# baurst/liso

Hardware: AMD Instinct MI355X
Metric: LISO train-step frames/sec (120k-pt clouds) (higher is better)
Workload: dtype bf16 (detector, BASELINE configs[2]) + f32 via bf16x3 MFMA (SLIM); north_star's 1e-3 on logits / flow is met by `parity_leg` (f32 via bf16x3 MFMA everywhere) and `fp32_exact_leg`, not by the bf16 detector

## Files before the change

include/liso_box_mining.h:

```cpp
#ifndef LISO_BOX_MINING_H
#define LISO_BOX_MINING_H

#include <stddef.h>
#include <stdint.h>

#ifdef __cplusplus
extern "C" {
#endif

size_t liso_scan_workspace_bytes(int batch, long n);
int liso_scan_inclusive_i32(const int32_t* in, int batch, long n, int32_t* out, void* workspace, size_t workspace_bytes,
                            void* stream);

int liso_mine_boxes_from_regions(const double* props, int batch, int k, const float* row_coords, int gx, const float* col_coords,
                                 int gy, float ppm_x, float ppm_y, float* center, double* dims, double* rot, float* dims_f32,
                                 float* rot_f32, void* stream);

typedef struct {
    int batch, k;
    int min_points;
    double aspect_ratio_max;
    double max_box_len_m;
    double min_box_area_m2;
    double min_box_volume_m3;
    int park_invalid;
} liso_mine_filter_cfg;

int liso_mine_filter_compact(const liso_mine_filter_cfg* cfg, const int64_t* num_labels, const float* center, const double* dims2,
                             const double* rot_in, const int64_t* num_pts, const float* fit_z, const float* fit_h, float* pos,
                             double* dims, double* rot, double* probs, double* velo, uint8_t* valid, int32_t* class_id,
                             int32_t* difficulty, int32_t* counts, float* kabsch_pos, float* kabsch_dims, float* kabsch_rot,
                             void* stream);

int liso_mine_box_motion(const double* trafos, int batch, int s, const float* pos, double* rot, double* velo, void* stream);

size_t liso_mine_nms_workspace_bytes(int batch, int k);
int liso_mine_nms_prepare(int batch, int k, int pre_nms_max, float* pos, double* dims, double* rot, double* probs, double* velo,
                          uint8_t* valid, int32_t* class_id, int32_t* difficulty, float* dense, uint8_t* enters, void* workspace,
                          size_t workspace_bytes, void* stream);

int liso_mine_nms_finish(int b, int k, int max_boxes, const int64_t* keep, const int32_t* num, const uint8_t* enters, float* pos,
                         double* dims, double* rot, double* probs, double* velo, uint8_t* valid, int32_t* class_id,
                         int32_t* difficulty, float* t_pos, float* t_dims, float* t_rot, uint8_t* t_valid, void* stream);

#ifdef __cplusplus
}
#endif
#endif
```

include/liso_flow_cluster.h:

```cpp
#ifndef LISO_FLOW_CLUSTER_H
#define LISO_FLOW_CLUSTER_H

#include <stddef.h>
#include <stdint.h>

#ifdef __cplusplus
extern "C" {
#endif

size_t liso_bev_dynamic_flow_workspace_bytes(int batch, int h, int w);

int liso_bev_dynamic_flow_f32(const float* points, int point_stride, const uint8_t* valid, const int32_t* pillar_coors,
                              const float* flow, int flow_stride, const double* odom_minus_eye, int batch, int n, int h,
                              int w, float* dynamicness, float* nonrigid_flow, void* workspace, size_t workspace_bytes,
                              void* stream);

int liso_odom_inverse_minus_eye_f64(const double* odom, int batch, double* out, void* stream);

size_t liso_fit_box_z_workspace_bytes(int n_points, int n_boxes);

int liso_fit_box_z_f32(const float* points, int point_stride, int n, const float* box_pos, int pos_dims,
                       const float* box_dims, int dims_dims, const float* box_rot, int k, float box_height,
                       int64_t* num_pts, float* fitted_z, float* fitted_height, void* workspace, size_t workspace_bytes,
                       void* stream);

typedef struct {
    int batch, gx, gy;
    int window;
    int min_samples;
    float eps;
    float flow_weight;
} liso_dbscan_cfg;

int liso_dbscan_components(const liso_dbscan_cfg* cfg, const uint8_t* dynamic_mask, const float* row_coords,
                           const float* col_coords, const float* flow, uint8_t* core, int32_t* parent, int32_t* is_root,
                           void* stream);

int liso_dbscan_labels(const liso_dbscan_cfg* cfg, const uint8_t* dynamic_mask, const float* row_coords, const float* col_coords,
                       const float* flow, const uint8_t* core, const int32_t* parent, const int32_t* root_rank,
                       int32_t* labels, void* stream);

int liso_region_props(const int32_t* labels, int batch, int gx, int gy, int max_labels, uint64_t* moments, double* props,
                      void* stream);

size_t liso_region_props_workspace_bytes(int batch, int gx, int gy, int max_labels);
int liso_region_props_ws(const int32_t* labels, int batch, int gx, int gy, int max_labels, uint64_t* moments, double* props,
                         void* workspace, size_t workspace_bytes, void* stream);

#ifdef __cplusplus
}
#endif
#endif
```

liso_amd/_lib.py:

```python
import ctypes
import os

import torch

_HERE = os.path.dirname(os.path.abspath(__file__))
LIB_PATH = os.path.join(_HERE, "libliso_hip.so")

_lib = None


class LisoHipError(RuntimeError):
    pass


_ERRORS = {-1: "LISO_EINVAL (bad pointer/size)", -2: "LISO_EWORKSPACE (workspace too small)",
           -3: "LISO_ELAUNCH (HIP launch failed)", -4: "LISO_GROUND_ELENGTH (int(67 / delta_R) > 255)"}


def _preload_torch_hip_runtime():
    tl = os.path.join(os.path.dirname(torch.__file__), "lib", "libamdhip64.so")
    if os.path.exists(tl):
        ctypes.CDLL(tl, mode=ctypes.RTLD_GLOBAL)


def lib():
    global _lib
    if _lib is None:
        if not os.path.exists(LIB_PATH):
            raise LisoHipError(
                f"{LIB_PATH} not found: build it with `python -c 'import __graft_entry__ as g; g.build()'` "
                "or `make -C liso_amd/csrc`.  liso_amd has no CPU fallback for device ops.")
        _preload_torch_hip_runtime()
        _lib = ctypes.CDLL(LIB_PATH)
        _declare(_lib)
    return _lib


def check(code, what):
    if code != 0:
        raise LisoHipError(f"{what} failed: {_ERRORS.get(code, code)}")


def stream_ptr(device=None):
    return ctypes.c_void_p(torch.cuda.current_stream(device).cuda_stream)


def ptr(t):
    return ctypes.c_void_p(t.data_ptr())


def multi_copy(pairs):
    import torch

    fast = []
    for d, s_ in pairs:
        if (d.is_cuda and s_.is_cuda and d.device == s_.device and d.dtype == s_.dtype and d.shape == s_.shape and d.is_contiguous()
                and s_.is_contiguous() and (not fast or fast[0][0].device == d.device)):
            if d.numel() and d.data_ptr() != s_.data_ptr():
                fast.append((d, s_))
        else:
            d.copy_(s_, non_blocking=True)
    if len(fast) == 1:
        fast[0][0].copy_(fast[0][1], non_blocking=True)
    elif fast:
        n = len(fast)
        dst = (ctypes.c_void_p * n)(*[d.data_ptr() for d, _ in fast])
        src = (ctypes.c_void_p * n)(*[s_.data_ptr() for _, s_ in fast])
        nb = (ctypes.c_size_t * n)(*[d.numel() * d.element_size() for d, _ in fast])
        with torch.cuda.device(fast[0][0].device):
            check(lib().liso_multi_copy(n, dst, src, nb, stream_ptr()), "multi_copy")


def copy_blocks(jobs):
    import torch

    n = len(jobs)
    if n == 0:
        return
    dst = (ctypes.c_void_p * n)()
    src = (ctypes.c_void_p * n)()
    rows = (ctypes.c_uint * n)()
    rb = (ctypes.c_uint * n)()
    ds = (ctypes.c_size_t * n)()
    ss = (ctypes.c_size_t * n)()

    def rows_view(t):
        assert t.dtype == torch.float32 and t.is_cuda
        if t.dim() == 1:
            assert t.stride(0) == 1 or t.numel() <= 1
            return 1, t.numel(), t.numel()
        inner = 1
        for k in range(t.dim() - 1, 0, -1):
            assert t.shape[k] == 1 or t.stride(k) == inner, (tuple(t.shape), t.stride())
            inner *= t.shape[k]
        return t.shape[0], inner, (t.stride(0) if t.shape[0] > 1 else inner)

    for i, (d, s_) in enumerate(jobs):
        assert tuple(d.shape) == tuple(s_.shape), (tuple(d.shape), tuple(s_.shape))
        r, c, dstr = rows_view(d)
        r2, c2, sstr = rows_view(s_)
        assert (r, c) == (r2, c2)
        dst[i], src[i], rows[i], rb[i], ds[i], ss[i] = d.data_ptr(), s_.data_ptr(), r, 4 * c, 4 * dstr, 4 * sstr
    with torch.cuda.device(jobs[0][0].device):
        check(lib().liso_multi_copy_rows(n, dst, src, rows, rb, ds, ss, stream_ptr()), "multi_copy_rows")


def require_cuda(*tensors):
    for t in tensors:
        if not t.is_cuda:
            raise LisoHipError("device op called with a CPU tensor; liso_amd has no CPU fallback")


_vp, _i, _f, _sz, _lg = ctypes.c_void_p, ctypes.c_int, ctypes.c_float, ctypes.c_size_t, ctypes.c_long

SIGNATURES = {
    "liso_iou3d_overlap_bev_f32": (_i, [_vp, _i, _vp, _i, _vp, _vp]),
    "liso_iou3d_iou_bev_f32": (_i, [_vp, _i, _vp, _i, _vp, _vp]),
    "liso_iou3d_nms_workspace_bytes": (_sz, [_i]),
    "liso_iou3d_nms_f32": (_i, [_vp, _i, _f, _vp, _vp, _vp, _sz, _vp]),
    "liso_iou3d_nms_normal_f32": (_i, [_vp, _i, _f, _vp, _vp, _vp, _sz, _vp]),
    "liso_iou3d_iou_bev_cpu_f32": (_i, [_vp, _i, _vp, _i, _vp]),
    "liso_pillars_voxelize_workspace_bytes": (_sz, [_vp, _i, _i]),
    "liso_pillars_voxelize_f32": (_i, [_vp, _vp, _i, _vp, _vp, _vp, _vp, _vp, _vp, _vp, _sz, _vp]),
    "liso_pfn_partials_bytes": (_sz, []),
    "liso_pfn_decorate_workspace_bytes": (_sz, [_i, _i]),
    "liso_pfn_decorate_f32": (_i, [_vp, _vp, _i, _vp, _vp, _vp, _vp, _vp, _vp, _vp, _vp, _sz, _vp]),
    "liso_pfn_bn_prepare_f32": (_i, [_vp, _vp, _vp, _i, _vp, _vp, _vp, _vp, _vp, _vp, _f, _f, _i, _vp, _vp, _vp, _vp]),
    "liso_pfn_forward_scatter": (_i, [_vp, _vp, _vp, _vp, _i, _vp, _vp, _vp, _vp, _i, _vp, _vp]),
    "liso_pfn_backward": (_i, [_vp, _vp, _vp, _vp, _i, _vp, _vp, _vp, _vp, _vp, _i, _vp, _i, _vp, _vp, _vp, _vp, _vp]),
    "liso_kabsch_workspace_bytes": (_sz, [_vp]),
    "liso_kabsch_trafos_f32": (_i, [_vp, _vp, _vp, _vp, _vp, _vp, _vp, _vp, _vp, _vp, _vp, _sz, _vp]),
    "liso_kabsch_trafos_counted_f32": (_i, [_vp, _vp, _vp, _vp, _vp, _vp, _vp, _vp, _vp, _vp, _vp, _vp, _sz, _vp]),
    "liso_symm_ortho_fwd_f64": (_i, [_vp, _i, _vp, _vp, _vp, _vp, _vp]),
    "liso_symm_ortho_bwd_f64": (_i, [_vp, _vp, _vp, _vp, _i, _vp, _vp]),
    "liso_weighted_moments_workspace_bytes": (_sz, [_i]),
    "liso_weighted_moments_fwd_f32": (_i, [_vp, _vp, _vp, _i, ctypes.c_long, _vp, _vp, _sz, _vp]),
    "liso_weighted_moments_bwd_f32": (_i, [_vp, _vp, _vp, _i, ctypes.c_long, _vp, _vp, _vp, _vp, _vp]),
    "liso_bev_dynamic_flow_workspace_bytes": (_sz, [_i, _i, _i]),
    "liso_bev_dynamic_flow_f32": (_i, [_vp, _i, _vp, _vp, _vp, _i, _vp, _i, _i, _i, _i, _vp, _vp, _vp, _sz, _vp]),
    "liso_odom_inverse_minus_eye_f64": (_i, [_vp, _i, _vp, _vp]),
    "liso_fit_box_z_workspace_bytes": (_sz, [_i, _i]),
    "liso_fit_box_z_f32": (_i, [_vp, _i, _i, _vp, _i, _vp, _i, _vp, _i, _f, _vp, _vp, _vp, _vp, _sz, _vp]),
    "liso_dbscan_components": (_i, [_vp, _vp, _vp, _vp, _vp, _vp, _vp, _vp, _vp]),
    "liso_dbscan_labels": (_i, [_vp, _vp, _vp, _vp, _vp, _vp, _vp, _vp, _vp, _vp]),
    "liso_region_props": (_i, [_vp, _i, _i, _i, _i, _vp, _vp, _vp]),
    "liso_region_props_workspace_bytes": (_sz, [_i, _i, _i, _i]),
    "liso_region_props_ws": (_i, [_vp, _i, _i, _i, _i, _vp, _vp, _vp, _sz, _vp]),
    "liso_corr_lookup_fwd_f32": (_i, [_vp, _vp, _vp, _vp, _vp, _vp]),
    "liso_corr_lookup_fwd_tiled_f32": (_i, [_vp, _vp, _vp, _vp, _vp, _vp]),
    "liso_corr_lookup_bwd_dvol_f32": (_i, [_vp, _vp, _vp, _vp, _vp]),
    "liso_corr_pyramid_fwd_f32": (_i, [_vp, _vp, _vp, _vp]),
    "liso_corr_pyramid_bwd_f32": (_i, [_vp, _vp, _vp, _vp]),
    "liso_corr_bwd_features_workspace_bytes": (_sz, [_vp]),
    "liso_corr_bwd_features_f32": (_i, [_vp, _i, _vp, _vp, _vp, _vp, _vp, _vp, _sz, _vp]),
    "liso_rows_combine_f32": (_i, [_lg, _i, _vp, _lg, _vp, _lg, _vp, _lg, _vp, _lg, _vp, _lg, _i, _vp]),
    "liso_gru_out_rows_train_f32": (_i, [_lg, _i, _vp, _lg, _vp, _vp, _lg, _vp, _lg, _vp]),
    "liso_gru_out_rows_bwd_f32": (_i, [_lg, _i, _vp, _lg, _vp, _vp, _lg, _vp, _lg, _vp, _lg, _vp, _vp, _vp]),
    "liso_gru_in_rows_bwd_f32": (_i, [_lg, _i, _vp, _lg, _vp, _lg, _vp, _vp, _vp, _lg, _vp, _lg, _vp, _vp]),
    "liso_raft_state_step_train_f32": (_i, [_i, _i, _vp, _vp, _vp, _vp, _vp, _vp, _vp, _vp, _vp]),
    "liso_raft_pack_output_grads_f32": (_i, [_lg, _i, _vp, _vp, _vp, _vp]),
    "liso_nearest_point_loss_fwd_f32": (_i, [_vp] * 8),
    "liso_nearest_point_loss_bwd_f32": (_i, [_vp] * 9),
    "liso_slim_decode_weights_fwd": (_i, [_vp] * 6 + [_i] + [_vp] * 4),
    "liso_slim_decode_weights_bwd": (_i, [_vp] * 9),
    "liso_slim_decode_points_fwd": (_i, [_vp] * 9),
    "liso_slim_decode_points_bwd": (_i, [_vp] * 11),
    "liso_slim_loss_workspace_bytes": (_sz, []),
    "liso_slim_static_points_loss_fwd": (_i, [_i, ctypes.c_long, _vp, _i, _vp, _vp, _vp, _vp, _vp, _vp, _sz, _vp]),
    "liso_slim_static_points_loss_bwd": (_i, [_i, ctypes.c_long, _vp, _i, _vp, _vp, _vp, _vp, _vp, _vp, _vp, _vp, _vp]),
    "liso_slim_knn_queries": (_i, [_i, _i, ctypes.c_long, _i, _vp, _i, _vp, _vp, _vp, _vp, _vp]),
    "liso_slim_nearest_point_loss_fwd": (_i, [_vp, _vp, _i, _vp, _vp, _vp, _i, _vp, _vp, _vp, _vp, _vp, _sz, _vp]),
    "liso_slim_nearest_point_loss_bwd": (_i, [_vp, _vp, _i, _vp, _vp, _vp, _i, _vp, _vp, _vp, _vp, _vp, _vp, _vp]),
    "liso_bev_gather_fwd_f32": (_i, [_vp, _vp, ctypes.c_long, _i, ctypes.c_float, _vp, _vp]),
    "liso_bev_gather_bwd_f32": (_i, [_vp, _vp, _vp, _vp, ctypes.c_long, _i, _vp, _vp, _vp]),
    "liso_gru_in_fwd_f32": (_i, [_vp, _vp, _vp, ctypes.c_long, _vp, _vp, _vp, _vp, _vp]),
    "liso_gru_in_bwd_f32": (_i, [_vp, _vp, ctypes.c_long, _vp, _vp, _vp, _vp, _vp, _vp, ctypes.c_long, _vp, _vp]),
    "liso_gru_out_fwd_f32": (_i, [ctypes.c_long, _vp, _vp, _vp, _vp, _vp]),
    "liso_gru_out_bwd_f32": (_i, [ctypes.c_long, _vp, _vp, _vp, _vp, _vp, _vp, _vp, _vp]),
    "liso_gru_in_rows_f32": (_i, [ctypes.c_long, _i, _vp, ctypes.c_long, _vp, ctypes.c_long, _vp, _vp, ctypes.c_long, _vp]),
    "liso_gru_out_rows_f32": (_i, [ctypes.c_long, _i, _vp, ctypes.c_long, _vp, _vp, ctypes.c_long, _vp]),
    "liso_multi_copy": (_i, [_i, _vp, _vp, _vp, _vp]),
    "liso_bev_lin_index": (_i, [_vp, _i, _vp, _i, ctypes.c_long, _i, _i, _vp, _vp]),
    "liso_channel_extrema_workspace_bytes": (_sz, []),
    "liso_channel_extrema_f32": (_i, [_vp, ctypes.c_long, _i, _i, _vp, _vp, _sz, _vp]),
    "liso_bev_plan_tile_lin": (_i, [_vp, _i, ctypes.c_long, _i, _i, _i, _i, _vp, _vp]),
    "liso_bev_plan_rank": (_i, [_vp, _vp, ctypes.c_long, _vp, _vp, _vp]),
    "liso_bev_plan_expand": (_i, [_vp, _vp, _vp, _i, ctypes.c_long, _i, _i, _i, _i, _vp, _vp, _vp, _vp]),
    "liso_raft_state_step_f32": (_i, [_i, _i, _vp, ctypes.c_long, _vp, _vp, _vp, _vp]),
    "liso_raft_upsample_scratch_bytes": (_sz, [_vp]),
    "liso_raft_upsample_outputs_fwd_f32": (_i, [_vp] * 5),
    "liso_raft_upsample_outputs_bwd_f32": (_i, [_vp, _vp, _vp, _sz, _vp, _vp, _vp]),
    "liso_centerloss_workspace_bytes": (_sz, [_vp]),
    "liso_centerloss_fwd_f32": (_i, [_vp] * 17 + [_sz, _vp]),
    "liso_centerloss_bwd_f32": (_i, [_vp] * 21),
    "liso_render_center_targets_f32": (_i, [_vp] * 12),
    "liso_conv_pack_weights_batched": (_i, [_vp, _i, _vp]),
    "liso_conv_in_finalize": (_i, [_vp, _i, _i, _i, _i, ctypes.c_long, _vp, _vp, _f, _vp, _vp]),
    "liso_residual_affine_relu_f32": (_i, [_vp, _vp, _vp, _i, _i, _vp, _vp, _vp, _i, _i, _vp, _i, ctypes.c_long, _i, _vp]),
    "liso_scan_workspace_bytes": (_sz, [_i, ctypes.c_long]),
    "liso_scan_inclusive_i32": (_i, [_vp, _i, ctypes.c_long, _vp, _vp, _sz, _vp]),
    "liso_mine_boxes_from_regions": (_i, [_vp, _i, _i, _vp, _i, _vp, _i, _f, _f, _vp, _vp, _vp, _vp, _vp, _vp]),
    "liso_mine_filter_compact": (_i, [_vp] * 21),
    "liso_mine_box_motion": (_i, [_vp, _i, _i, _vp, _vp, _vp, _vp]),
    "liso_mine_nms_workspace_bytes": (_sz, [_i, _i]),
    "liso_mine_nms_prepare": (_i, [_i, _i, _i] + [_vp] * 11 + [_sz, _vp]),
    "liso_mine_nms_finish": (_i, [_i, _i, _i] + [_vp] * 16),
    "liso_adamw_step_f32": (_i, [_vp, _vp, _vp, _vp, _sz] + [ctypes.c_double] * 5 + [ctypes.c_long, _vp]),
    "liso_adamw_step_scaled_f32": (_i, [_vp, _vp, _vp, _vp, _sz] + [ctypes.c_double] * 6 + [ctypes.c_long, _vp]),
    "liso_grad_nonfinite_f32": (_i, [_vp, _sz, _vp, _vp]),
    "liso_adamw_step_amp_f32": (_i, [_vp, _vp, _vp, _vp, _sz] + [ctypes.c_double] * 6 + [_vp, _vp]),
    "liso_loss_scale_update": (_i, [_vp, ctypes.c_double, ctypes.c_double, _i, _vp]),
    "liso_rmsprop_step_f32": (_i, [_vp, _vp, _vp, _sz] + [ctypes.c_double] * 4 + [_vp]),
    "liso_multi_copy_rows": (_i, [_i, _vp, _vp, _vp, _vp, _vp, _vp, _vp]),
    "liso_gather_f32": (_i, [_i, _vp, _vp, _vp, _vp]),
    "liso_bn_workspace_bytes": (_sz, [_i]),
    "liso_bn_relu_fwd": (_i, [_vp, _i, ctypes.c_long, _i, _vp, _vp, _vp, _vp, _f, _f, _i, _i, _vp, _vp, _vp, _sz, _vp]),
    "liso_in_workspace_bytes": (_sz, [_i, _i]),
    "liso_in_relu_fwd": (_i, [_vp, _i, _i, ctypes.c_long, _i, _vp, _vp, _f, _i, _vp, _vp, _vp, _sz, _vp]),
    "liso_in_relu_bwd": (_i, [_vp, _vp, _i, _i, ctypes.c_long, _i, _vp, _vp, _i, _vp, _vp, _vp, _vp, _sz, _vp]),
    "liso_in_relu_bwd_sum": (_i, [_vp, _vp, _i, _i, ctypes.c_long, _i, _vp, _vp, _i, _vp, _vp, _vp, _vp, _sz, _vp]),
    "liso_bn_relu_bwd": (_i, [_vp, _vp, _i, ctypes.c_long, _i, _vp, _vp, _i, _i, _vp, _vp, _vp, _vp, _sz, _vp]),
    "liso_bn_relu_bwd_strided": (_i, [_vp, ctypes.c_long, _vp, ctypes.c_long, _i, ctypes.c_long, _i, _vp, _vp, _i, _i, _vp, ctypes.c_long, _vp, _vp, _vp, _sz, _vp]),
    "liso_bn_relu_bwd_chained": (_i, [_vp, ctypes.c_long, _vp, ctypes.c_long, _i, ctypes.c_long, _i, _vp, _vp, _i, _i, _vp, ctypes.c_long, _vp, _vp, _vp, _sz, _vp, _vp]),
    "liso_knn_workspace_bytes": (_sz, [_vp, _i]),
    "liso_knn_build_f32": (_i, [_vp, _vp, _i, _i, _vp, _sz, _vp]),
    "liso_knn_sorted_ids": (_i, [_vp, _vp, _i, _vp, _vp]),
    "liso_knn_query_f32": (_i, [_vp, _vp, _vp, _vp, _i, _vp, _i, _i, _vp, _vp, _i, _vp]),
    "liso_conv_packed_bytes": (_sz, [_i, _i, _i, _i]),
    "liso_conv_pack_weights": (_i, [_vp, _i, _i, _i, _i, _i, _i, _i, _vp, _vp]),
    "liso_conv_stats_rows": (_i, [_vp]),
    "liso_conv_kernel_kind": (_i, [_vp]),
    "liso_conv_forward": (_i, [_vp] * 10),
    "liso_conv_set_option": (_i, [_i, _i]),
    "liso_conv_forward_sparse": (_i, [_vp] * 11),
    "liso_conv_plan_info": (_i, [_vp, _vp]),
    "liso_conv_wgrad_workspace_bytes": (_sz, [_vp]),
    "liso_conv_wgrad": (_i, [_vp, _vp, _vp, _vp, _vp, _i, _i, _vp, _vp, _vp, _sz, _vp]),
    "liso_conv_wgrad_deferred": (_i, [_vp, _vp, _vp, _vp, _vp, _i, _i, _vp, _vp, _vp, _sz, _vp, _vp]),
    "liso_conv_wgrad_reduce": (_i, [_vp, _vp]),
    "liso_conv_wgrad_sparse_workspace_bytes": (_sz, [_vp]),
    "liso_conv_wgrad_sparse_f32": (_i, [_vp, _vp, _vp, _vp, _i, _vp, _vp, _vp, _sz, _vp]),
    "liso_conv_wgrad_smallci_workspace_bytes": (_sz, [_i, _i, _i, _i, _i]),
    "liso_conv_wgrad_smallci_f32": (_i, [_vp, ctypes.c_long, _vp, ctypes.c_long, _i, _i, _i, _i, _i, _vp, _vp, _vp, _sz, _vp]),
    "liso_sparse_conv_stat_groups": (_i, [_i, _i, _i]),
    "liso_sparse_conv_workspace_bytes": (_sz, [_i, _i, _i, _i, _i, _i, _i]),
    "liso_sparse_conv_forward": (_i, [_vp, ctypes.c_long, _i, _vp, _vp, _vp, _i, _i, _i, _i, _i, _i, _i, _vp, _vp, _vp, _vp, _vp, _sz, _vp]),
    "liso_sparse_conv_dgrad": (_i, [_vp, ctypes.c_long, _i, _vp, _vp, _i, _i, _i, _i, _i, _i, _vp, ctypes.c_long, _vp, _vp, _sz, _i, _vp]),
    "liso_sparse_stem_workspace_bytes": (_sz, [_i, _i, _i, _i]),
    "liso_sparse_stem_forward_f32": (_i, [_vp, ctypes.c_long, _vp, _vp, _vp, _i, _i, _i, _i, _i, _vp, _vp, _vp, _vp, _sz, _vp]),
    "liso_conv_bn_finalize": (_i, [_vp, _i, _i, _i, ctypes.c_long, _vp, _vp, _vp, _vp, _vp, _f, _f, _vp, _vp]),
    "liso_points_in_boxes_workspace_bytes": (_sz, [_vp]),
    "liso_points_in_boxes_f32": (_i, [_vp] * 9 + [_sz, _vp]),
    "liso_match_greedy_f32": (_i, [_vp, ctypes.c_long, ctypes.c_long, _i, _i, _vp, _f, _vp, _vp, _vp, _vp, _vp, _vp, _vp]),
    "liso_fit_boxes_closeness_workspace_bytes": (_sz, [ctypes.c_long, _i]),
    "liso_fit_boxes_closeness_f32": (_i, [_vp, ctypes.c_long, _i, _vp, _vp, _i, _f, _vp, _vp, _vp, _sz, _vp]),
    "liso_bike_rollout_fwd_f32": (_i, [_i, _i, _vp, _vp, _vp, _vp, _f, _f, _f, _vp, _vp]),
    "liso_bike_rollout_bwd_f32": (_i, [_i, _i, _vp, _vp, _vp, _f, _f, _f, _vp, _vp, _vp, _vp, _vp, _vp]),
    "liso_smooth_tracks_jerk_f32": (_i, [_vp, _vp, _i, _i, _i, _f, _f, _vp, _vp]),
    "liso_flow_metrics_state_bytes": (_sz, []),
    "liso_flow_metrics_result_bytes": (_sz, []),
    "liso_flow_metrics_reset": (_i, [_vp, _vp]),
    "liso_flow_metrics_update": (_i, [_vp, _lg, _vp, _lg, _vp, _lg, _i, _vp, _lg, _vp, _lg, _vp, _lg, _vp, _vp, _vp, _vp, _i, _vp, _vp]),
    "liso_flow_metrics_read": (_i, [_vp, _vp, _vp]),
    "liso_det_nms_workspace_bytes": (_sz, [_i, _i]),
    "liso_det_nms_order": (_i, [_i, _i, _vp, _vp, _vp, _f, _vp, _vp, _vp, _sz, _vp]),
    "liso_det_nms_select": (_i, [_i, _i, _vp, _vp, _vp, _f, _i, _i, _vp, _vp, _vp]),
    "liso_det_nms_gather": (_i, [_i, _i, _i, _vp, _vp, _vp, _i, _vp]),
    "liso_ground_jcp_workspace_bytes": (_sz, [_vp]),
    "liso_ground_jcp_f32": (_i, [_vp, _vp, _vp, _vp, _vp, _sz, _vp]),
    "liso_ground_jcp_stages_f32": (_i, [_vp, _vp, _vp, _vp, _vp, _sz, _i, _i, _vp]),
    "liso_ground_cone_f32": (_i, [_i, _i, _i, _vp, _vp, ctypes.c_double, ctypes.c_double, _vp, _vp, _vp]),
    "liso_ground_compact_workspace_bytes": (_sz, [_i, _i]),
    "liso_ground_compact_f32": (_i, [_i, _i, _i, _vp, _vp, _vp, _vp, _vp, _vp, _sz, _vp]),
    "liso_bev_free_mask_workspace_bytes": (_sz, [_i, _i]),
    "liso_bev_free_mask": (_i, [_vp, ctypes.c_long, _i, _i, _i, _vp, _vp, _vp, _sz, _vp]),
    "liso_bev_select_free_cells": (_i, [_vp, _vp, _i, _i, _vp, _i, _vp, _vp]),
    "liso_snippet_paste": (_i, [_vp, ctypes.c_long, _vp, _vp, _vp, _vp, ctypes.c_double, ctypes.c_double, _i, _vp, _vp, _vp, _vp]),
    "liso_sample_transform_f32": (_i, [_i, _i, _i] + [_vp] * 7),
    "liso_sample_transform_poses_f64": (_i, [_i, _vp, _vp, _i, _vp, _i, _vp]),
    "liso_bev_crop_workspace_bytes": (_sz, [_i, _i]),
    "liso_bev_crop_f32": (_i, [_vp] * 14 + [_sz, _vp]),
    "liso_bev_point_maps_workspace_bytes": (_sz, [_i, _i, _i, _i]),
    "liso_bev_point_maps_f32": (_i, [_i] * 5 + [_vp] * 6 + [ctypes.c_double] + [_vp] * 5 + [_sz, _vp]),
    "liso_box_has_points_f32": (_i, [_i] * 4 + [_vp] * 7),
    "liso_filter_boxes": (_i, [_vp] * 6 + [_i] + [_vp] * 3),
    "liso_object_velocity_f64": (_i, [_i, _i] + [_vp] * 5),
    "liso_ignore_region_mask": (_i, [_i] * 4 + [ctypes.c_double] * 2 + [_vp] * 6),
    "liso_render_center_targets_ex_f32": (_i, [_vp] * 15),
    "liso_snippet_cut_workspace_bytes": (_sz, [_i, _i, _i]),
    "liso_snippet_cut_f32": (_i, [_i, _i, _i, _vp, _vp, _vp, _i, _vp, _vp, _lg] + [_vp] * 5 + [_sz, _vp]),
    "liso_track_sequences_workspace_bytes": (_sz, [_i, _i, _i, _i]),
    "liso_track_sequences": (_i, [_i] * 4 + [_vp] * 7 + [ctypes.c_double] + [_vp] * 10 + [_sz, _vp]),
}


CONV_MAX_TAPS, CONV_MAX_CLASSES, CONV_BF16, CONV_F32X3, CONV_F32, CONV_F16 = 49, 4, 0, 1, 2, 3
ELEM_F32, ELEM_BF16, ELEM_F16 = 0, 1, 2
_ELEM_CODES = {torch.float32: ELEM_F32, torch.bfloat16: ELEM_BF16, torch.float16: ELEM_F16}
LOSS_SCALE_STATE_BYTES = 32


def elem_code(dtype):
    code = _ELEM_CODES.get(dtype)
    if code is None:
        raise TypeError(f"no device kernel takes {dtype} tensors (float32, bfloat16 or float16)")
    return code


def is_half(dtype):
    return elem_code(dtype) != ELEM_F32
CONV_OPT_SHARED_GPU = 1
CONV_OPT_ROLES_CUS = 2


class ConvDesc(ctypes.Structure):
    _fields_ = [("batch", _i), ("hi", _i), ("wi", _i), ("ci", _i), ("x_pix_stride", _i), ("ho", _i), ("wo", _i), ("co", _i),
                ("y_pix_stride", _i), ("y_ch_off", _i), ("hv", _i), ("wv", _i), ("isy", _i), ("isx", _i), ("osy", _i), ("osx", _i),
                ("n_classes", _i), ("class_tap_begin", _i * (CONV_MAX_CLASSES + 1)), ("class_ooy", _i * CONV_MAX_CLASSES),
                ("class_oox", _i * CONV_MAX_CLASSES), ("n_taps", _i), ("tap_dy", _i * CONV_MAX_TAPS), ("tap_dx", _i * CONV_MAX_TAPS),
                ("tap_w", _i * CONV_MAX_TAPS), ("w_taps", _i), ("mode", _i), ("out_f32", _i), ("in_relu", _i), ("out_relu", _i),
                ("in_affine_batch_stride", _i), ("wgrad_co", _i)]


class ConvPackJob(ctypes.Structure):
    _fields_ = [("src", _vp), ("dst", _vp), ("d0", _i), ("d1", _i), ("kh", _i), ("kw", _i), ("transposed", _i), ("for_dgrad", _i),
                ("mode", _i)]


class WgradReduceJob(ctypes.Structure):
    _fields_ = [("slab", _vp), ("bias_slab", _vp), ("dw", _vp), ("dbias", _vp), ("cip", ctypes.c_long), ("cop", ctypes.c_long),
                ("splits", _i), ("bias_rows", _i), ("taps", _i), ("ci", _i), ("co", _i), ("transposed", _i)]


class KnnGrid(ctypes.Structure):
    _fields_ = [("x_min", _f), ("y_min", _f), ("cell", _f), ("nx", _i), ("ny", _i), ("z_min", _f), ("z_cell", _f), ("nz", _i)]


class CenterLossCfg(ctypes.Structure):
    _fields_ = [("batch", _i), ("h", _i), ("w", _i), ("res_x", _f), ("res_y", _f), ("z_min", _f), ("z_max", _f),
                ("sup_weight", _f), ("rot_reg_weight", _f)]


class NpLossCfg(ctypes.Structure):
    _fields_ = [("batch", _i), ("n", ctypes.c_long), ("n_b", ctypes.c_long), ("ext", _f * 4), ("fov_mode", _i), ("delta", _f)]


class SlimDecodeCfg(ctypes.Structure):
    _fields_ = [("samples", _i), ("n", ctypes.c_long), ("h", _i), ("w", _i), ("logit_mode", _i * 4), ("static_flow_zero", _i),
                ("dynamic_flow_zero", _i), ("overwrite_flow", _i), ("overwrite_logits", _i), ("non_rigid", _i), ("use_static_aggr", _i),
                ("dyn_grad_scale", _f), ("ext_lo", ctypes.c_double * 2), ("ext_span", ctypes.c_double * 2)]


class SlimDecodeOut(ctypes.Structure):
    FIELDS = ("dis_logit", "dis", "logits", "probs", "staticness", "dynamicness", "groundness", "dyn_flow", "stat_flow", "agg_flow", "saf_flow")
    _fields_ = [(k, _vp) for k in FIELDS] + [("flags", _vp)]


class SlimNpLossCfg(ctypes.Structure):
    _fields_ = [("samples", _i), ("clouds", _i), ("n", ctypes.c_long), ("n_b", ctypes.c_long), ("ext", _f * 4), ("fov_mode", _i), ("delta", _f)]


class BoxPtsCfg(ctypes.Structure):
    _fields_ = [("batch", _i), ("n", ctypes.c_long), ("k", _i), ("point_stride", _i), ("precision", _i), ("dims_bloat", _f)]


class GruCfg(ctypes.Structure):
    _fields_ = [("batch", _i), ("ch", _i), ("cx", _i), ("hw", ctypes.c_long)]


class UpsampleCfg(ctypes.Structure):
    _fields_ = [("n_it", _i), ("batch2", _i), ("dirs", _i), ("h", _i), ("w", _i), ("factor", _i), ("flow_scale", _f)]


class MineFilterCfg(ctypes.Structure):
    _fields_ = [("batch", _i), ("k", _i), ("min_points", _i), ("aspect_ratio_max", ctypes.c_double), ("max_box_len_m", ctypes.c_double),
                ("min_box_area_m2", ctypes.c_double), ("min_box_volume_m3", ctypes.c_double), ("park_invalid", _i)]


class DetGatherField(ctypes.Structure):
    _fields_ = [("src", _vp), ("dst", _vp), ("row_elems", _i), ("elem_bytes", _i), ("pad_bits", ctypes.c_uint64)]


class GroundCfg(ctypes.Structure):
    _fields_ = [("batch", _i), ("n_max", _i), ("point_stride", _i), ("width", _i), ("height", _i),
                ("sensor_height", ctypes.c_double), ("delta_r", ctypes.c_double)]


class TargetsCfg(ctypes.Structure):
    _fields_ = [("batch", _i), ("n_boxes", _i), ("h", _i), ("w", _i), ("range_x", _f), ("range_y", _f)]


class DbscanCfg(ctypes.Structure):
    _fields_ = [("batch", _i), ("gx", _i), ("gy", _i), ("window", _i), ("min_samples", _i), ("eps", _f), ("flow_weight", _f)]


class CorrCfg(ctypes.Structure):
    _fields_ = [("batch", _i), ("h", _i), ("w", _i), ("dim", _i), ("levels", _i), ("radius", _i)]


class KabschCfg(ctypes.Structure):
    _fields_ = [("batch", _i), ("n_points", _i), ("n_slots", _i), ("point_stride", _i), ("flow_stride", _i),
                ("slope", _f), ("scale_fg", _f), ("scale_bg", _f), ("softness", _i)]


class PillarCfg(ctypes.Structure):
    _fields_ = [("x_min", _f), ("y_min", _f), ("z_min", _f), ("vx", _f), ("vy", _f), ("vz", _f), ("gx", _i),
                ("gy", _i), ("max_points", _i), ("max_voxels", _i), ("n_channels", _i)]


class _Everything:
    def __contains__(self, name):
        return True


class KernelTimer:

    def __init__(self):
        self.enabled = set()
        self.events = {}
        self.units = {}
        self.bytes = {}
        self.weights = {}
        self.weight = 1.0

    def enable(self, name):
        self.enabled.add(name)
        self.events.setdefault(name, [])

    def enable_all(self):
        self.enabled = _Everything()

    def disable_all(self):
        self.enabled = set()

    def launch(self, name, fn, units=None, nbytes=None):
        if name not in self.enabled:
            return fn()
        a, b = torch.cuda.Event(enable_timing=True), torch.cuda.Event(enable_timing=True)
        a.record()
        r = fn()
        b.record()
        self.events.setdefault(name, []).append((a, b))
        self.weights.setdefault(name, []).append(float(self.weight))
        if units is not None:
            self.units.setdefault(name, []).append(units)
        if nbytes is not None:
            self.bytes.setdefault(name, []).append(nbytes)
        return r

    def mean_units(self, name):
        u = self.units.get(name, [])
        return sum(u) / len(u) if u else None

    def durations_ms(self, name):
        torch.cuda.synchronize()
        return [a.elapsed_time(b) for a, b in self.events.get(name, [])]

    def weighted_total_ms(self, name):
        return sum(d * w for d, w in zip(self.durations_ms(name), self.weights.get(name, [])))

    def reset(self):
        for k in self.events:
            self.events[k] = []
        self.units = {}
        self.bytes = {}
        self.weights = {}


TIMER = KernelTimer()


def _declare(l):
    for name, (res, args) in SIGNATURES.items():
        fn = getattr(l, name)
        fn.restype = res
        fn.argtypes = args
```

liso_amd/csrc/box_mining.hip:

```cpp
#include <hip/hip_runtime.h>
#include <math.h>
#include <stdint.h>

#include "../../include/liso_box_mining.h"
#include "../../include/liso_iou3d.h"
#include "dev_common.h"

namespace {

using liso_dev::check_launch;

constexpr int kScanThreads = 256;
constexpr int kScanPer = 8;
constexpr int kScanChunk = kScanThreads * kScanPer;
constexpr int32_t kUnknownClass = 2147483647;
constexpr int32_t kInvalidClass = kUnknownClass - 1;

__device__ __forceinline__ int block_exclusive_scan(int v, int* total) {
    __shared__ int wsum[kScanThreads / 64];
    const int lane = threadIdx.x & 63, wave = threadIdx.x >> 6;
    int inc = v;
#pragma unroll
    for (int d = 1; d < 64; d <<= 1) {
        const int o = __shfl_up(inc, d, 64);
        if (lane >= d) inc += o;
    }
    if (lane == 63) wsum[wave] = inc;
    __syncthreads();
    int base = 0, tot = 0;
#pragma unroll
    for (int w = 0; w < kScanThreads / 64; w++) {
        if (w < wave) base += wsum[w];
        tot += wsum[w];
    }
    __syncthreads();
    *total = tot;
    return base + inc - v;
}

__global__ __launch_bounds__(kScanThreads) void scan_block_sums_kernel(const int32_t* __restrict__ in, long n, int nblk,
                                                                       int32_t* __restrict__ sums) {
    const long row = blockIdx.y, base = (long)blockIdx.x * kScanChunk + (long)threadIdx.x * kScanPer;
    const int32_t* p = in + row * n;
    int s = 0;
#pragma unroll
    for (int e = 0; e < kScanPer; e++)
        if (base + e < n) s += p[base + e];
    int tot;
    block_exclusive_scan(s, &tot);
    if (threadIdx.x == 0) sums[row * nblk + blockIdx.x] = tot;
}

__global__ __launch_bounds__(kScanThreads) void scan_sums_kernel(int32_t* __restrict__ sums, int nblk) {
    int32_t* p = sums + (long)blockIdx.x * nblk;
    int carry = 0;
    for (int c0 = 0; c0 < nblk; c0 += kScanThreads) {
        const int i = c0 + threadIdx.x;
        const int v = i < nblk ? p[i] : 0;
        int tot;
        const int ex = block_exclusive_scan(v, &tot);
        if (i < nblk) p[i] = carry + ex;
        carry += tot;
    }
}

__global__ __launch_bounds__(kScanThreads) void scan_apply_kernel(const int32_t* __restrict__ in, long n, int nblk,
                                                                  const int32_t* __restrict__ offs, int32_t* __restrict__ out) {
    const long row = blockIdx.y, base = (long)blockIdx.x * kScanChunk + (long)threadIdx.x * kScanPer;
    const int32_t* p = in + row * n;
    int v[kScanPer], s = 0;
#pragma unroll
    for (int e = 0; e < kScanPer; e++) {
        v[e] = base + e < n ? p[base + e] : 0;
        s += v[e];
    }
    int tot;
    int run = block_exclusive_scan(s, &tot) + offs[row * nblk + blockIdx.x];
    int32_t* q = out + row * n;
#pragma unroll
    for (int e = 0; e < kScanPer; e++) {
        run += v[e];
        if (base + e < n) q[base + e] = run;
    }
}

__global__ void boxes_from_regions_kernel(const double* __restrict__ props, long total, const float* __restrict__ row_coords, int gx,
                                          const float* __restrict__ col_coords, int gy, double ppm_x, double ppm_y,
                                          float* __restrict__ center, double* __restrict__ dims, double* __restrict__ rot,
                                          float* __restrict__ dims_f32, float* __restrict__ rot_f32) {
    const long i = (long)blockIdx.x * blockDim.x + threadIdx.x;
    if (i >= total) return;
    const double* p = props + i * 5;
    const long hi = (gx < gy ? gx : gy) - 1;
    long r = (long)p[0], c = (long)p[1];
    r = r < 0 ? 0 : (r > hi ? hi : r);
    c = c < 0 ? 0 : (c > hi ? hi : c);
    center[i * 2 + 0] = row_coords[r];
    center[i * 2 + 1] = col_coords[c];
    const double d0 = p[3] * 1.0 / ppm_x, d1 = p[4] * 1.0 / ppm_y;
    dims[i * 2 + 0] = d0;
    dims[i * 2 + 1] = d1;
    rot[i] = p[2];
    dims_f32[i * 2 + 0] = (float)d0;
    dims_f32[i * 2 + 1] = (float)d1;
    rot_f32[i] = (float)p[2];
}

__global__ __launch_bounds__(64) void filter_compact_kernel(const liso_mine_filter_cfg c, const int64_t* __restrict__ num_labels,
                                                            const float* __restrict__ center, const double* __restrict__ dims2,
                                                            const double* __restrict__ rot_in, const int64_t* __restrict__ num_pts,
                                                            const float* __restrict__ fit_z, const float* __restrict__ fit_h,
                                                            float* __restrict__ pos, double* __restrict__ dims, double* __restrict__ rot,
                                                            double* __restrict__ probs, double* __restrict__ velo,
                                                            uint8_t* __restrict__ valid, int32_t* __restrict__ class_id,
                                                            int32_t* __restrict__ difficulty, int32_t* __restrict__ counts,
                                                            float* __restrict__ kpos, float* __restrict__ kdims, float* __restrict__ krot) {
    const int b = blockIdx.x, lane = threadIdx.x, K = c.k;
    const long o = (long)b * K;
    const long nl = num_labels[b];
    int run = 0;
    for (int k0 = 0; k0 < K; k0 += 64) {
        const int k = k0 + lane;
        bool ok = false;
        double d0 = 0.0, d1 = 0.0, hz = 0.0, th = 0.0;
        float cx = 0.f, cy = 0.f, fz = 0.f;
        if (k < K) {
            d0 = dims2[(o + k) * 2];
            d1 = dims2[(o + k) * 2 + 1];
            hz = (double)fit_h[o + k];
            th = rot_in[o + k];
            cx = center[(o + k) * 2];
            cy = center[(o + k) * 2 + 1];
            fz = fit_z[o + k];
            const bool exists = k < nl;
            const bool enough = num_pts[o + k] >= (int64_t)c.min_points;
            const double aspect = d0 / fmax(d1, 0.001);
            const bool aspect_ok = aspect <= c.aspect_ratio_max;
            const bool not_large = d0 <= c.max_box_len_m;
            const bool foot_ok = d0 * d1 > c.min_box_area_m2;
            const bool vol_ok = (d0 * d1) * hz > c.min_box_volume_m3;
            ok = exists && enough && aspect_ok && not_large && foot_ok && vol_ok;
        }
        const unsigned long long m = __ballot(ok);
        const int dst = run + __popcll(m & ((1ull << lane) - 1ull));
        if (ok) {
            const long q = o + dst;
            pos[q * 3] = cx, pos[q * 3 + 1] = cy, pos[q * 3 + 2] = fz;
            dims[q * 3] = d0, dims[q * 3 + 1] = d1, dims[q * 3 + 2] = hz;
            rot[q] = th;
            probs[q] = 1.0;
            velo[q] = 0.0;
            valid[q] = 1;
            class_id[q] = kUnknownClass;
            difficulty[q] = 1;
            kpos[q * 3] = cx, kpos[q * 3 + 1] = cy, kpos[q * 3 + 2] = fz;
            kdims[q * 3] = (float)d0, kdims[q * 3 + 1] = (float)d1, kdims[q * 3 + 2] = (float)hz;
            krot[q] = (float)th;
        }
        run += __popcll(m);
    }
    for (int k = run + lane; k < K; k += 64) {
        const long q = o + k;
        pos[q * 3] = 0.f, pos[q * 3 + 1] = 0.f, pos[q * 3 + 2] = 0.f;
        dims[q * 3] = 0.0, dims[q * 3 + 1] = 0.0, dims[q * 3 + 2] = 0.0;
        rot[q] = 0.0, probs[q] = 0.0, velo[q] = 0.0;
        valid[q] = 0;
        class_id[q] = kInvalidClass;
        difficulty[q] = kInvalidClass;
        const float park = c.park_invalid ? 1e6f : 0.f;
        kpos[q * 3] = park, kpos[q * 3 + 1] = park, kpos[q * 3 + 2] = park;
        kdims[q * 3] = 0.f, kdims[q * 3 + 1] = 0.f, kdims[q * 3 + 2] = 0.f;
        krot[q] = 0.f;
    }
    if (lane == 0) counts[b] = run;
}

struct Aff {
    double a[3][3], t[3];
};

__device__ __forceinline__ Aff aff_load(const double* __restrict__ m) {
    Aff r;
#pragma unroll
    for (int i = 0; i < 3; i++) {
#pragma unroll
        for (int j = 0; j < 3; j++) r.a[i][j] = m[i * 4 + j];
        r.t[i] = m[i * 4 + 3];
    }
    return r;
}

__device__ __forceinline__ Aff aff_mul(const Aff& x, const Aff& y) {
    Aff r;
#pragma unroll
    for (int i = 0; i < 3; i++) {
#pragma unroll
        for (int j = 0; j < 3; j++) r.a[i][j] = x.a[i][0] * y.a[0][j] + x.a[i][1] * y.a[1][j] + x.a[i][2] * y.a[2][j];
        r.t[i] = x.a[i][0] * y.t[0] + x.a[i][1] * y.t[1] + x.a[i][2] * y.t[2] + x.t[i];
    }
    return r;
}

__device__ __forceinline__ Aff aff_inv(const Aff& x) {
    Aff r;
    const double (*a)[3] = x.a;
    const double c00 = a[1][1] * a[2][2] - a[1][2] * a[2][1], c01 = a[1][2] * a[2][0] - a[1][0] * a[2][2],
                 c02 = a[1][0] * a[2][1] - a[1][1] * a[2][0];
    const double det = a[0][0] * c00 + a[0][1] * c01 + a[0][2] * c02;
    const double id = 1.0 / det;
    r.a[0][0] = c00 * id;
    r.a[1][0] = c01 * id;
    r.a[2][0] = c02 * id;
    r.a[0][1] = (a[0][2] * a[2][1] - a[0][1] * a[2][2]) * id;
    r.a[1][1] = (a[0][0] * a[2][2] - a[0][2] * a[2][0]) * id;
    r.a[2][1] = (a[0][1] * a[2][0] - a[0][0] * a[2][1]) * id;
    r.a[0][2] = (a[0][1] * a[1][2] - a[0][2] * a[1][1]) * id;
    r.a[1][2] = (a[0][2] * a[1][0] - a[0][0] * a[1][2]) * id;
    r.a[2][2] = (a[0][0] * a[1][1] - a[0][1] * a[1][0]) * id;
#pragma unroll
    for (int i = 0; i < 3; i++) r.t[i] = -(r.a[i][0] * x.t[0] + r.a[i][1] * x.t[1] + r.a[i][2] * x.t[2]);
    return r;
}

__global__ void box_motion_kernel(const double* __restrict__ trafos, int batch, int s, const float* __restrict__ pos,
                                  double* __restrict__ rot, double* __restrict__ velo) {
    const int i = blockIdx.x * blockDim.x + threadIdx.x;
    if (i >= batch * s) return;
    const int b = i / s, k = i - b * s;
    const double* base = trafos + (long)b * (s + 1) * 16;
    const Aff fg = aff_load(base + (long)k * 16), bg = aff_load(base + (long)s * 16);
    const double th = rot[i];
    Aff box;
    const double cs = cos(th), sn = sin(th);
    box.a[0][0] = cs, box.a[0][1] = -sn, box.a[0][2] = 0.0;
    box.a[1][0] = sn, box.a[1][1] = cs, box.a[1][2] = 0.0;
    box.a[2][0] = 0.0, box.a[2][1] = 0.0, box.a[2][2] = 1.0;
    box.t[0] = (double)pos[(long)i * 3], box.t[1] = (double)pos[(long)i * 3 + 1], box.t[2] = (double)pos[(long)i * 3 + 2];
    const Aff m = aff_mul(aff_mul(aff_inv(box), aff_inv(bg)), aff_mul(fg, box));
    rot[i] = th + atan2(m.t[1], m.t[0]);
    velo[i] = sqrt(m.t[0] * m.t[0] + m.t[1] * m.t[1] + m.t[2] * m.t[2]);
}

struct Slot {
    double dims[3], rot, probs, velo;
    float pos[3];
    int32_t class_id, difficulty;
    uint8_t valid, pad[3];
};

__global__ __launch_bounds__(64) void nms_prepare_kernel(int k, int pre_nms_max, float* __restrict__ pos, double* __restrict__ dims,
                                                         double* __restrict__ rot, double* __restrict__ probs, double* __restrict__ velo,
                                                         uint8_t* __restrict__ valid, int32_t* __restrict__ class_id,
                                                         int32_t* __restrict__ difficulty, float* __restrict__ dense,
                                                         uint8_t* __restrict__ enters, Slot* __restrict__ scratch) {
    const int b = blockIdx.x, lane = threadIdx.x;
    const long o = (long)b * k;
    Slot* sc = scratch + o;
    for (int i = lane; i < k; i += 64) {
        Slot s;
        const long q = o + i;
        s.pos[0] = pos[q * 3], s.pos[1] = pos[q * 3 + 1], s.pos[2] = pos[q * 3 + 2];
        s.dims[0] = dims[q * 3], s.dims[1] = dims[q * 3 + 1], s.dims[2] = dims[q * 3 + 2];
        s.rot = rot[q], s.probs = probs[q], s.velo = velo[q];
        s.class_id = class_id[q], s.difficulty = difficulty[q], s.valid = valid[q];
        s.pad[0] = s.pad[1] = s.pad[2] = 0;
        sc[i] = s;
    }
    __syncthreads();
    for (int i = lane; i < k; i += 64) {
        const bool vi = sc[i].valid != 0;
        double ki = vi ? sc[i].probs : -(double)INFINITY;
        ki = ki != ki ? -(double)INFINITY : ki;
        int rank = 0;
        for (int j = 0; j < k; j++) {
            double kj = sc[j].valid ? sc[j].probs : -(double)INFINITY;
            kj = kj != kj ? -(double)INFINITY : kj;
            rank += (kj > ki || (kj == ki && j < i)) ? 1 : 0;
        }
        const Slot s = sc[i];
        const long q = o + rank;
        pos[q * 3] = s.pos[0], pos[q * 3 + 1] = s.pos[1], pos[q * 3 + 2] = s.pos[2];
        dims[q * 3] = s.dims[0], dims[q * 3 + 1] = s.dims[1], dims[q * 3 + 2] = s.dims[2];
        rot[q] = s.rot, probs[q] = s.probs, velo[q] = s.velo;
        class_id[q] = s.class_id, difficulty[q] = s.difficulty, valid[q] = s.valid;
        const bool in = vi && (pre_nms_max <= 0 || rank < pre_nms_max);
        enters[q] = in ? 1 : 0;
        float* dn = dense + q * 7;
        if (in) {
            dn[0] = s.pos[0], dn[1] = s.pos[1], dn[2] = s.pos[2];
            dn[3] = (float)s.dims[0], dn[4] = (float)s.dims[1], dn[5] = (float)s.dims[2];
            dn[6] = (float)s.rot;
        } else {
            dn[0] = 1e6f + 10.0f * (float)rank, dn[1] = 1e6f, dn[2] = 0.f;
            dn[3] = 1e-3f, dn[4] = 1e-3f, dn[5] = 1e-3f, dn[6] = 0.f;
        }
    }
}

constexpr int kMaxNmsSlots = 16384;

__global__ __launch_bounds__(64) void nms_finish_kernel(int b, int k, int max_boxes, const int64_t* __restrict__ keep,
                                                        const int32_t* __restrict__ num, const uint8_t* __restrict__ enters,
                                                        float* __restrict__ pos, double* __restrict__ dims, double* __restrict__ rot,
                                                        double* __restrict__ probs, double* __restrict__ velo, uint8_t* __restrict__ valid,
                                                        int32_t* __restrict__ class_id, int32_t* __restrict__ difficulty,
                                                        float* __restrict__ t_pos, float* __restrict__ t_dims, float* __restrict__ t_rot,
                                                        uint8_t* __restrict__ t_valid) {
    __shared__ uint8_t hit[kMaxNmsSlots];
    const int lane = threadIdx.x;
    const long o = (long)b * k;
    for (int i = lane; i < k; i += 64) hit[i] = 0;
    __syncthreads();
    const int n = min(max(num[0], 0), k);
    for (int i = lane; i < n; i += 64) {
        const long j = keep[i];
        if (j >= 0 && j < k) hit[j] = 1;
    }
    __syncthreads();
    int run = 0;
    for (int k0 = 0; k0 < k; k0 += 64) {
        const int i = k0 + lane;
        const bool kept = i < k && hit[i] && enters[o + i] && valid[o + i];
        const unsigned long long m = __ballot(kept);
        const int rank = run + __popcll(m & ((1ull << lane) - 1ull)) + 1;
        run += __popcll(m);
        if (i >= k) continue;
        const bool ok = kept && rank <= max_boxes;
        const long q = o + i;
        if (!ok) {
            pos[q * 3] = 0.f, pos[q * 3 + 1] = 0.f, pos[q * 3 + 2] = 0.f;
            dims[q * 3] = 0.0, dims[q * 3 + 1] = 0.0, dims[q * 3 + 2] = 0.0;
            rot[q] = 0.0, probs[q] = 0.0, velo[q] = 0.0;
            class_id[q] = kInvalidClass, difficulty[q] = kInvalidClass;
        }
        valid[q] = ok ? 1 : 0;
        t_valid[q] = ok ? 1 : 0;
        t_pos[q * 3] = pos[q * 3], t_pos[q * 3 + 1] = pos[q * 3 + 1], t_pos[q * 3 + 2] = pos[q * 3 + 2];
#pragma unroll
        for (int e = 0; e < 3; e++) t_dims[q * 3 + e] = fmaxf((float)dims[q * 3 + e], 1e-3f);
        t_rot[q] = (float)rot[q];
    }
}

}

extern "C" {

size_t liso_scan_workspace_bytes(int batch, long n) {
    if (batch <= 0 || n <= 0) return 0;
    const long nblk = (n + kScanChunk - 1) / kScanChunk;
    return (size_t)batch * nblk * sizeof(int32_t);
}

int liso_scan_inclusive_i32(const int32_t* in, int batch, long n, int32_t* out, void* workspace, size_t workspace_bytes,
                            void* stream) {
    if (!in || !out || !workspace || batch <= 0 || n <= 0) return LISO_EINVAL;
    if (workspace_bytes < liso_scan_workspace_bytes(batch, n)) return LISO_EWORKSPACE;
    const long nblk = (n + kScanChunk - 1) / kScanChunk;
    if (nblk > 65535l * 64) return LISO_EINVAL;
    hipStream_t st = (hipStream_t)stream;
    int32_t* sums = (int32_t*)workspace;
    scan_block_sums_kernel<<<dim3((unsigned)nblk, batch), kScanThreads, 0, st>>>(in, n, (int)nblk, sums);
    scan_sums_kernel<<<batch, kScanThreads, 0, st>>>(sums, (int)nblk);
    scan_apply_kernel<<<dim3((unsigned)nblk, batch), kScanThreads, 0, st>>>(in, n, (int)nblk, sums, out);
    return check_launch();
}

int liso_mine_boxes_from_regions(const double* props, int batch, int k, const float* row_coords, int gx, const float* col_coords,
                                 int gy, float ppm_x, float ppm_y, float* center, double* dims, double* rot, float* dims_f32,
                                 float* rot_f32, void* stream) {
    if (!props || !row_coords || !col_coords || !center || !dims || !rot || !dims_f32 || !rot_f32) return LISO_EINVAL;
    if (batch <= 0 || k <= 0 || gx <= 0 || gy <= 0) return LISO_EINVAL;
    const long total = (long)batch * k;
    boxes_from_regions_kernel<<<(unsigned)((total + 127) / 128), 128, 0, (hipStream_t)stream>>>(
        props, total, row_coords, gx, col_coords, gy, (double)ppm_x, (double)ppm_y, center, dims, rot, dims_f32, rot_f32);
    return check_launch();
}

int liso_mine_filter_compact(const liso_mine_filter_cfg* cfg, const int64_t* num_labels, const float* center, const double* dims2,
                             const double* rot_in, const int64_t* num_pts, const float* fit_z, const float* fit_h, float* pos,
                             double* dims, double* rot, double* probs, double* velo, uint8_t* valid, int32_t* class_id,
                             int32_t* difficulty, int32_t* counts, float* kabsch_pos, float* kabsch_dims, float* kabsch_rot,
                             void* stream) {
    if (!cfg || cfg->batch <= 0 || cfg->k <= 0) return LISO_EINVAL;
    if (!num_labels || !center || !dims2 || !rot_in || !num_pts || !fit_z || !fit_h || !pos || !dims || !rot || !probs || !velo ||
        !valid || !class_id || !difficulty || !counts || !kabsch_pos || !kabsch_dims || !kabsch_rot)
        return LISO_EINVAL;
    filter_compact_kernel<<<cfg->batch, 64, 0, (hipStream_t)stream>>>(*cfg, num_labels, center, dims2, rot_in, num_pts, fit_z, fit_h, pos,
                                                                     dims, rot, probs, velo, valid, class_id, difficulty, counts,
                                                                     kabsch_pos, kabsch_dims, kabsch_rot);
    return check_launch();
}

int liso_mine_box_motion(const double* trafos, int batch, int s, const float* pos, double* rot, double* velo, void* stream) {
    if (!trafos || !pos || !rot || !velo || batch <= 0 || s <= 0) return LISO_EINVAL;
    const int total = batch * s;
    box_motion_kernel<<<(total + 63) / 64, 64, 0, (hipStream_t)stream>>>(trafos, batch, s, pos, rot, velo);
    return check_launch();
}

size_t liso_mine_nms_workspace_bytes(int batch, int k) {
    if (batch <= 0 || k <= 0) return 0;
    return (size_t)batch * k * sizeof(Slot);
}

int liso_mine_nms_prepare(int batch, int k, int pre_nms_max, float* pos, double* dims, double* rot, double* probs, double* velo,
                          uint8_t* valid, int32_t* class_id, int32_t* difficulty, float* dense, uint8_t* enters, void* workspace,
                          size_t workspace_bytes, void* stream) {
    if (batch <= 0 || k <= 0 || !pos || !dims || !rot || !probs || !velo || !valid || !class_id || !difficulty || !dense || !enters ||
        !workspace)
        return LISO_EINVAL;
    if (workspace_bytes < liso_mine_nms_workspace_bytes(batch, k)) return LISO_EWORKSPACE;
    if (((uintptr_t)workspace & 7) != 0) return LISO_EINVAL;
    nms_prepare_kernel<<<batch, 64, 0, (hipStream_t)stream>>>(k, pre_nms_max, pos, dims, rot, probs, velo, valid, class_id, difficulty,
                                                             dense, enters, (Slot*)workspace);
    return check_launch();
}

int liso_mine_nms_finish(int b, int k, int max_boxes, const int64_t* keep, const int32_t* num, const uint8_t* enters, float* pos,
                         double* dims, double* rot, double* probs, double* velo, uint8_t* valid, int32_t* class_id,
                         int32_t* difficulty, float* t_pos, float* t_dims, float* t_rot, uint8_t* t_valid, void* stream) {
    if (b < 0 || k <= 0 || k > kMaxNmsSlots || !keep || !num || !enters || !pos || !dims || !rot || !probs || !velo || !valid ||
        !class_id || !difficulty || !t_pos || !t_dims || !t_rot || !t_valid)
        return LISO_EINVAL;
    nms_finish_kernel<<<1, 64, 0, (hipStream_t)stream>>>(b, k, max_boxes, keep, num, enters, pos, dims, rot, probs, velo, valid, class_id,
                                                        difficulty, t_pos, t_dims, t_rot, t_valid);
    return check_launch();
}

}
```

liso_amd/csrc/flow_cluster.hip:

```cpp
#include <hip/hip_runtime.h>
#include "zero_fill.h"
#include <math.h>
#include <stdint.h>

#include "../../include/liso_flow_cluster.h"
#include "../../include/liso_iou3d.h"
#include "dev_common.h"

namespace {

using liso_dev::check_launch;

constexpr double kFix = 16777216.0;

__global__ __launch_bounds__(256) void bev_scatter_kernel(const float* __restrict__ points, int ps, const uint8_t* __restrict__ valid,
                                   const int32_t* __restrict__ coors, const float* __restrict__ flow, int fs,
                                   const double* __restrict__ ome, int batch, int n, int h, int w,
                                   long long* __restrict__ sums, int* __restrict__ counts) {
    const size_t i = (size_t)blockIdx.x * blockDim.x + threadIdx.x;
    const int lane = threadIdx.x & 63;
    long long cell = -1;
    long long q[4] = {0, 0, 0, 0};
    if (i < (size_t)batch * n && valid[i]) {
        const int b = (int)(i / n);
        const int r = coors[i * 2 + 0], c = coors[i * 2 + 1];
        if (r >= 0 && r < h && c >= 0 && c < w) {
            const float* p = points + i * ps;
            const float* f = flow + i * fs;
            const double* M = ome + (size_t)b * 16;
            const double x = p[0], y = p[1], z = p[2];
            float nr[3];
#pragma unroll
            for (int k = 0; k < 3; k++) {
                const float stat = (float)(M[k * 4 + 0] * x + M[k * 4 + 1] * y + M[k * 4 + 2] * z + M[k * 4 + 3]);
                nr[k] = f[k] - stat;
            }
            const float len = sqrtf(nr[0] * nr[0] + nr[1] * nr[1] + nr[2] * nr[2]);
            cell = (long long)(((size_t)b * h + r) * w + c);
            q[0] = llrint((double)len * kFix);
            q[1] = llrint((double)nr[0] * kFix);
            q[2] = llrint((double)nr[1] * kFix);
            q[3] = llrint((double)nr[2] * kFix);
        }
    }
    const long long prev = __shfl_up(cell, 1);
    const bool head = lane == 0 || prev != cell;
    const unsigned long long heads = __ballot(head);
    const int run = __popcll(heads & ((2ull << lane) - 1ull));
    int cnt = cell >= 0 ? 1 : 0;
#pragma unroll
    for (int o = 1; o < 64; o <<= 1) {
        const int other_run = __shfl_down(run, o);
        const bool take = lane + o < 64 && other_run == run;
#pragma unroll
        for (int k = 0; k < 4; k++) {
            const long long v = __shfl_down(q[k], o);
            if (take) q[k] += v;
        }
        const int vc = __shfl_down(cnt, o);
        if (take) cnt += vc;
    }
    if (!head || cell < 0) return;
    unsigned long long* s = (unsigned long long*)(sums + cell * 4);
    atomicAdd(s + 0, (unsigned long long)q[0]);
    atomicAdd(s + 1, (unsigned long long)q[1]);
    atomicAdd(s + 2, (unsigned long long)q[2]);
    atomicAdd(s + 3, (unsigned long long)q[3]);
    atomicAdd(&counts[cell], cnt);
}

__global__ void bev_mean_kernel(const long long* __restrict__ sums, const int* __restrict__ counts, size_t cells,
                                float* __restrict__ dyn, float* __restrict__ nrflow) {
    const size_t i = (size_t)blockIdx.x * blockDim.x + threadIdx.x;
    if (i >= cells) return;
    const int cnt = counts[i];
    float v[4];
#pragma unroll
    for (int k = 0; k < 4; k++) {
        v[k] = (float)((double)sums[i * 4 + k] / kFix);
        if (cnt > 1) v[k] = v[k] / (float)cnt;
    }
    dyn[i] = v[0];
    nrflow[i * 3 + 0] = v[1]; nrflow[i * 3 + 1] = v[2]; nrflow[i * 3 + 2] = v[3];
}

constexpr int kFitThreads = 256;
constexpr int kFitTile = 256;
constexpr int kFitMaxBlocks = 256;

struct FitPartial {
    int count;
    float zmin, zmax, zmin_sensor;
    int zmin_idx;
};

__global__ __launch_bounds__(kFitThreads) void fit_z_kernel(const float* __restrict__ points, int ps, int n,
                                                            const float* __restrict__ box_pos, int pos_dims,
                                                            const float* __restrict__ box_dims, int dims_dims,
                                                            const float* __restrict__ box_rot, int k, float box_height,
                                                            FitPartial* __restrict__ partials, int tiles_per_block) {
    __shared__ float px[kFitTile], py[kFitTile], pz[kFitTile];
    __shared__ FitPartial red[kFitThreads / 64][64];
    const int tid = threadIdx.x, lane = tid & 63, wave = tid >> 6;
    const int box = blockIdx.y * 64 + lane;
    const bool has = box < k;
    double bx = 0, by = 0, bz = 0, c = 1, s = 0;
    float hx = 0, hy = 0, hz = 0;
    if (has) {
        bx = box_pos[box * pos_dims + 0]; by = box_pos[box * pos_dims + 1];
        bz = pos_dims == 3 ? (double)box_pos[box * pos_dims + 2] : 0.0;
        const double th = (double)box_rot[box];
        c = cos(th); s = sin(th);
        hx = 0.5f * box_dims[box * dims_dims + 0]; hy = 0.5f * box_dims[box * dims_dims + 1];
        hz = 0.5f * (dims_dims == 3 ? box_dims[box * dims_dims + 2] : box_height);
    }
    FitPartial acc = {0, box_height, -box_height, 0.f, 0x7fffffff};
    const int tile0 = blockIdx.x * tiles_per_block;
    for (int t = 0; t < tiles_per_block; t++) {
        const int base = (tile0 + t) * kFitTile;
        if (base >= n) break;
        {
            const int i = base + tid;
            if (i < n) { px[tid] = points[(size_t)i * ps]; py[tid] = points[(size_t)i * ps + 1]; pz[tid] = points[(size_t)i * ps + 2]; }
        }
        __syncthreads();
        const int cntp = n - base < kFitTile ? n - base : kFitTile;
        if (has) {
            for (int j = wave; j < cntp; j += kFitThreads / 64) {
                const double dx = (double)px[j] - bx, dy = (double)py[j] - by;
                const float lx = (float)(c * dx + s * dy), ly = (float)(-s * dx + c * dy), lz = (float)((double)pz[j] - bz);
                if (fabsf(lx) < hx && fabsf(ly) < hy && fabsf(lz) < hz) {
                    acc.count++;
                    acc.zmax = fmaxf(acc.zmax, lz);
                    const int gi = base + j;
                    if (lz < acc.zmin || (lz == acc.zmin && gi < acc.zmin_idx)) { acc.zmin = lz; acc.zmin_sensor = pz[j]; acc.zmin_idx = gi; }
                }
            }
        }
        __syncthreads();
    }
    red[wave][lane] = acc;
    __syncthreads();
    if (wave == 0 && has) {
        FitPartial r = red[0][lane];
        for (int wv = 1; wv < kFitThreads / 64; wv++) {
            const FitPartial o = red[wv][lane];
            r.count += o.count;
            r.zmax = fmaxf(r.zmax, o.zmax);
            if (o.zmin < r.zmin || (o.zmin == r.zmin && o.zmin_idx < r.zmin_idx)) { r.zmin = o.zmin; r.zmin_sensor = o.zmin_sensor; r.zmin_idx = o.zmin_idx; }
        }
        partials[(size_t)blockIdx.x * k + box] = r;
    }
}

__global__ __launch_bounds__(64) void fit_z_final_kernel(const FitPartial* __restrict__ partials, int nblk, int k,
                                                         const float* __restrict__ points, int ps, int n, float box_height,
                                                         long long* __restrict__ num_pts, float* __restrict__ fz,
                                                         float* __restrict__ fh) {
    const int box = blockIdx.x, lane = threadIdx.x;
    if (box >= k) return;
    FitPartial r = {0, box_height, -box_height, 0.f, 0x7fffffff};
    for (int b = lane; b < nblk; b += 64) {
        const FitPartial o = partials[(size_t)b * k + box];
        r.count += o.count;
        r.zmax = fmaxf(r.zmax, o.zmax);
        if (o.zmin < r.zmin || (o.zmin == r.zmin && o.zmin_idx < r.zmin_idx)) { r.zmin = o.zmin; r.zmin_sensor = o.zmin_sensor; r.zmin_idx = o.zmin_idx; }
    }
#pragma unroll
    for (int off = 32; off > 0; off >>= 1) {
        FitPartial o;
        o.count = __shfl_xor(r.count, off);
        o.zmin = __shfl_xor(r.zmin, off);
        o.zmax = __shfl_xor(r.zmax, off);
        o.zmin_sensor = __shfl_xor(r.zmin_sensor, off);
        o.zmin_idx = __shfl_xor(r.zmin_idx, off);
        r.count += o.count;
        r.zmax = fmaxf(r.zmax, o.zmax);
        if (o.zmin < r.zmin || (o.zmin == r.zmin && o.zmin_idx < r.zmin_idx)) { r.zmin = o.zmin; r.zmin_sensor = o.zmin_sensor; r.zmin_idx = o.zmin_idx; }
    }
    if (lane != 0) return;
    const float height = fminf(fmaxf(r.zmax - r.zmin, 1.0f), 2.0f);
    const float zlow = r.count > 0 ? r.zmin_sensor : (n > 0 ? points[2] : 0.f);
    num_pts[box] = r.count;
    fh[box] = height;
    fz[box] = zlow + 0.5f * height;
}

__global__ void odom_inverse_minus_eye_kernel(const double* __restrict__ m_all, int batch, double* __restrict__ out_all) {
    const int b = blockIdx.x * blockDim.x + threadIdx.x;
    if (b >= batch) return;
    const double* m = m_all + (size_t)b * 16;
    double* o = out_all + (size_t)b * 16;
    const double a00 = m[0], a01 = m[1], a02 = m[2], a03 = m[3], a10 = m[4], a11 = m[5], a12 = m[6], a13 = m[7];
    const double a20 = m[8], a21 = m[9], a22 = m[10], a23 = m[11], a30 = m[12], a31 = m[13], a32 = m[14], a33 = m[15];
    const double s0 = a00 * a11 - a10 * a01, s1 = a00 * a12 - a10 * a02, s2 = a00 * a13 - a10 * a03;
    const double s3 = a01 * a12 - a11 * a02, s4 = a01 * a13 - a11 * a03, s5 = a02 * a13 - a12 * a03;
    const double c5 = a22 * a33 - a32 * a23, c4 = a21 * a33 - a31 * a23, c3 = a21 * a32 - a31 * a22;
    const double c2 = a20 * a33 - a30 * a23, c1 = a20 * a32 - a30 * a22, c0 = a20 * a31 - a30 * a21;
    const double inv = 1.0 / (s0 * c5 - s1 * c4 + s2 * c3 + s3 * c2 - s4 * c1 + s5 * c0);
    o[0] = (a11 * c5 - a12 * c4 + a13 * c3) * inv - 1.0;
    o[1] = (-a01 * c5 + a02 * c4 - a03 * c3) * inv;
    o[2] = (a31 * s5 - a32 * s4 + a33 * s3) * inv;
    o[3] = (-a21 * s5 + a22 * s4 - a23 * s3) * inv;
    o[4] = (-a10 * c5 + a12 * c2 - a13 * c1) * inv;
    o[5] = (a00 * c5 - a02 * c2 + a03 * c1) * inv - 1.0;
    o[6] = (-a30 * s5 + a32 * s2 - a33 * s1) * inv;
    o[7] = (a20 * s5 - a22 * s2 + a23 * s1) * inv;
    o[8] = (a10 * c4 - a11 * c2 + a13 * c0) * inv;
    o[9] = (-a00 * c4 + a01 * c2 - a03 * c0) * inv;
    o[10] = (a30 * s4 - a31 * s2 + a33 * s0) * inv - 1.0;
    o[11] = (-a20 * s4 + a21 * s2 - a23 * s0) * inv;
    o[12] = (-a10 * c3 + a11 * c1 - a12 * c0) * inv;
    o[13] = (a00 * c3 - a01 * c1 + a02 * c0) * inv;
    o[14] = (-a30 * s3 + a31 * s1 - a32 * s0) * inv;
    o[15] = (a20 * s3 - a21 * s1 + a22 * s0) * inv - 1.0;
}

inline int fit_blocks(int n) {
    const int tiles = (n + kFitTile - 1) / kFitTile;
    return tiles < kFitMaxBlocks ? (tiles > 0 ? tiles : 1) : kFitMaxBlocks;
}

}

extern "C" {

size_t liso_bev_dynamic_flow_workspace_bytes(int batch, int h, int w) {
    if (batch <= 0 || h <= 0 || w <= 0) return 0;
    return (size_t)batch * h * w * (4 * sizeof(long long) + sizeof(int));
}

int liso_bev_dynamic_flow_f32(const float* points, int point_stride, const uint8_t* valid, const int32_t* pillar_coors,
                              const float* flow, int flow_stride, const double* odom_minus_eye, int batch, int n, int h,
                              int w, float* dynamicness, float* nonrigid_flow, void* workspace, size_t workspace_bytes,
                              void* stream) {
    if (batch <= 0 || n < 0 || h <= 0 || w <= 0 || point_stride < 3 || flow_stride < 3) return LISO_EINVAL;
    if (!dynamicness || !nonrigid_flow || !workspace || !odom_minus_eye) return LISO_EINVAL;
    if (n > 0 && (!points || !valid || !pillar_coors || !flow)) return LISO_EINVAL;
    const size_t need = liso_bev_dynamic_flow_workspace_bytes(batch, h, w);
    if (workspace_bytes < need) return LISO_EWORKSPACE;
    hipStream_t st = (hipStream_t)stream;
    const size_t cells = (size_t)batch * h * w;
    long long* sums = (long long*)workspace;
    int* counts = (int*)(sums + cells * 4);
    if (liso_zero::zero_async(workspace, need, st) != hipSuccess) return LISO_ELAUNCH;
    const size_t total = (size_t)batch * n;
    if (total > 0)
        bev_scatter_kernel<<<(unsigned)((total + 255) / 256), 256, 0, st>>>(points, point_stride, valid, pillar_coors, flow,
                                                                          flow_stride, odom_minus_eye, batch, n, h, w, sums,
                                                                          counts);
    bev_mean_kernel<<<(unsigned)((cells + 255) / 256), 256, 0, st>>>(sums, counts, cells, dynamicness, nonrigid_flow);
    return check_launch();
}

int liso_odom_inverse_minus_eye_f64(const double* odom, int batch, double* out, void* stream) {
    if (batch < 0 || (batch > 0 && (!odom || !out))) return LISO_EINVAL;
    if (batch == 0) return LISO_OK;
    odom_inverse_minus_eye_kernel<<<(batch + 63) / 64, 64, 0, (hipStream_t)stream>>>(odom, batch, out);
    return check_launch();
}

size_t liso_fit_box_z_workspace_bytes(int n_points, int n_boxes) {
    if (n_points < 0 || n_boxes <= 0) return 0;
    return (size_t)fit_blocks(n_points) * n_boxes * sizeof(FitPartial);
}

int liso_fit_box_z_f32(const float* points, int point_stride, int n, const float* box_pos, int pos_dims,
                       const float* box_dims, int dims_dims, const float* box_rot, int k, float box_height,
                       int64_t* num_pts, float* fitted_z, float* fitted_height, void* workspace, size_t workspace_bytes,
                       void* stream) {
    if (n < 0 || k < 0 || point_stride < 3 || (pos_dims != 2 && pos_dims != 3) || (dims_dims != 2 && dims_dims != 3))
        return LISO_EINVAL;
    if (k == 0) return LISO_OK;
    if (!box_pos || !box_dims || !box_rot || !num_pts || !fitted_z || !fitted_height || !workspace || (n > 0 && !points))
        return LISO_EINVAL;
    if (workspace_bytes < liso_fit_box_z_workspace_bytes(n, k)) return LISO_EWORKSPACE;
    hipStream_t st = (hipStream_t)stream;
    const int nblk = fit_blocks(n);
    const int tiles = (n + kFitTile - 1) / kFitTile;
    const int tpb = (tiles + nblk - 1) / nblk > 0 ? (tiles + nblk - 1) / nblk : 1;
    fit_z_kernel<<<dim3(nblk, (k + 63) / 64), kFitThreads, 0, st>>>(points, point_stride, n, box_pos, pos_dims, box_dims,
                                                                    dims_dims, box_rot, k, box_height,
                                                                    (FitPartial*)workspace, tpb);
    fit_z_final_kernel<<<k, 64, 0, st>>>((const FitPartial*)workspace, nblk, k, points, point_stride, n,
                                                     box_height, (long long*)num_pts, fitted_z, fitted_height);
    return check_launch();
}

}
```

liso_amd/csrc/flow_dbscan.hip:

```cpp
#include <hip/hip_runtime.h>
#include "zero_fill.h"
#include <math.h>
#include <stdint.h>
#include <stdlib.h>

#include "../../include/liso_flow_cluster.h"
#include "../../include/liso_iou3d.h"
#include "dev_common.h"

namespace {

using liso_dev::check_launch;

struct Cfg {
    int batch, gx, gy, win, min_samples;
    double eps_sqr;
    float flow_weight;
};

__device__ __forceinline__ double dist_sqr(const float* __restrict__ xs, const float* __restrict__ ys,
                                           const float* __restrict__ flow, float fw, int r0, int c0, size_t i0, int r1, int c1,
                                           size_t i1) {
    const double d0 = (double)xs[r0] - (double)xs[r1];
    const double d1 = (double)ys[c0] - (double)ys[c1];
    const double d2 = (double)(fw * flow[3 * i0 + 0]) - (double)(fw * flow[3 * i1 + 0]);
    const double d3 = (double)(fw * flow[3 * i0 + 1]) - (double)(fw * flow[3 * i1 + 1]);
    const double d4 = (double)(fw * flow[3 * i0 + 2]) - (double)(fw * flow[3 * i1 + 2]);
    return d0 * d0 + d1 * d1 + d2 * d2 + d3 * d3 + d4 * d4;
}

template <typename F>
__device__ __forceinline__ void for_each_neighbour(const Cfg& c, const uint8_t* __restrict__ dyn, const float* __restrict__ xs,
                                                   const float* __restrict__ ys, const float* __restrict__ flow, int b, int r,
                                                   int col, F&& f) {
    const size_t base = (size_t)b * c.gx * c.gy;
    const size_t me = base + (size_t)r * c.gy + col;
    const int r_lo = max(r - c.win, 0), r_hi = min(r + c.win, c.gx - 1);
    const int c_lo = max(col - c.win, 0), c_hi = min(col + c.win, c.gy - 1);
    for (int rr = r_lo; rr <= r_hi; rr++)
        for (int cc = c_lo; cc <= c_hi; cc++) {
            const size_t nb = base + (size_t)rr * c.gy + cc;
            if (!dyn[nb]) continue;
            if (dist_sqr(xs, ys, flow, c.flow_weight, r, col, me, rr, cc, nb) <= c.eps_sqr) f(nb);
        }
}

constexpr int kDenseWave = 20;

template <typename F>
__device__ __forceinline__ void wave_for_each_neighbour(const Cfg& c, const uint8_t* __restrict__ dyn, const float* __restrict__ xs,
                                                        const float* __restrict__ ys, const float* __restrict__ flow, size_t me,
                                                        int lane, F&& f) {
    const size_t per = (size_t)c.gx * c.gy;
    const int b = (int)(me / per), r = (int)((me % per) / c.gy), col = (int)(me % c.gy);
    const size_t base = (size_t)b * per;
    const int r_lo = max(r - c.win, 0), r_hi = min(r + c.win, c.gx - 1);
    const int c_lo = max(col - c.win, 0), c_hi = min(col + c.win, c.gy - 1);
    const int wc = c_hi - c_lo + 1, n = (r_hi - r_lo + 1) * wc;
    for (int k = lane; k < n; k += 64) {
        const int rr = r_lo + k / wc, cc = c_lo + k % wc;
        const size_t nb = base + (size_t)rr * c.gy + cc;
        if (dyn[nb] && dist_sqr(xs, ys, flow, c.flow_weight, r, col, me, rr, cc, nb) <= c.eps_sqr) f(nb);
    }
}

__global__ __launch_bounds__(256) void dbscan_core_kernel(Cfg c, const uint8_t* __restrict__ dyn, const float* __restrict__ xs,
                                                          const float* __restrict__ ys, const float* __restrict__ flow,
                                                          uint8_t* __restrict__ core, int* __restrict__ parent) {
    const size_t i = (size_t)blockIdx.x * blockDim.x + threadIdx.x;
    const size_t per = (size_t)c.gx * c.gy, total = per * c.batch;
    const int lane = threadIdx.x & 63;
    const bool flagged = i < total && dyn[i];
    unsigned long long todo = __ballot(flagged);
    int is_core = 0;
    if (__popcll(todo) > kDenseWave) {
        if (flagged) {
            int count = 0;
            for_each_neighbour(c, dyn, xs, ys, flow, (int)(i / per), (int)((i % per) / c.gy), (int)(i % c.gy), [&](size_t) { count++; });
            is_core = count >= c.min_samples;
        }
        todo = 0ull;
    }
    while (todo) {
        const int src = __ffsll((long long)todo) - 1;
        todo &= todo - 1;
        int count = 0;
        wave_for_each_neighbour(c, dyn, xs, ys, flow, i - lane + src, lane, [&](size_t) { count++; });
#pragma unroll
        for (int o = 32; o > 0; o >>= 1) count += __shfl_xor(count, o);
        if (lane == src) is_core = count >= c.min_samples;
    }
    if (i >= total) return;
    core[i] = (uint8_t)is_core;
    parent[i] = is_core ? (int)(i % per) : -1;
}

__device__ __forceinline__ int find_root(const int* parent, int x) {
    int p = __hip_atomic_load(&parent[x], __ATOMIC_RELAXED, __HIP_MEMORY_SCOPE_AGENT);
    while (p != x) { x = p; p = __hip_atomic_load(&parent[x], __ATOMIC_RELAXED, __HIP_MEMORY_SCOPE_AGENT); }
    return x;
}

__device__ __forceinline__ int find_root_compress(int* parent, int x0) {
    const int r = find_root(parent, x0);
    if (r != x0) atomicMin(&parent[x0], r);
    return r;
}

__global__ __launch_bounds__(256) void dbscan_union_kernel(Cfg c, const uint8_t* __restrict__ dyn, const uint8_t* __restrict__ core,
                                                           const float* __restrict__ xs, const float* __restrict__ ys,
                                                           const float* __restrict__ flow, int* __restrict__ parent) {
    const size_t i = (size_t)blockIdx.x * blockDim.x + threadIdx.x;
    const size_t per = (size_t)c.gx * c.gy, total = per * c.batch;
    const int lane = threadIdx.x & 63;
    unsigned long long todo = __ballot(i < total && core[i]);
    if (__popcll(todo) > kDenseWave) {
        if (i < total && core[i]) {
            const int b = (int)(i / per), r = (int)((i % per) / c.gy), col = (int)(i % c.gy);
            int* par = parent + (size_t)b * per;
            const int me = (int)(i % per);
            for_each_neighbour(c, dyn, xs, ys, flow, b, r, col, [&](size_t nb) {
                if (!core[nb]) return;
                const int other = (int)(nb % per);
                if (other >= me) return;
                int x = me, y = other;
                while (true) {
                    x = find_root_compress(par, x);
                    y = find_root_compress(par, y);
                    if (x == y) break;
                    if (x < y) { const int t = x; x = y; y = t; }
                    const int old = atomicMin(&par[x], y);
                    if (old == x) break;
                    x = old;
                }
            });
        }
        return;
    }
    while (todo) {
        const int src = __ffsll((long long)todo) - 1;
        todo &= todo - 1;
        const size_t cell = i - lane + src;
        int* par = parent + (cell / per) * per;
        const int me = (int)(cell % per);
        wave_for_each_neighbour(c, dyn, xs, ys, flow, cell, lane, [&](size_t nb) {
            if (!core[nb]) return;
            const int other = (int)(nb % per);
            if (other >= me) return;
            int x = me, y = other;
            while (true) {
                x = find_root_compress(par, x);
                y = find_root_compress(par, y);
                if (x == y) break;
                if (x < y) { const int t = x; x = y; y = t; }
                const int old = atomicMin(&par[x], y);
                if (old == x) break;
                x = old;
            }
        });
    }
}

constexpr int kTR = 16, kTC = 32, kUfThreads = 256, kMaxWin = 8;
constexpr int kRegMax = (kTR + 2 * kMaxWin) * (kTC + 2 * kMaxWin);

__device__ __forceinline__ int lds_find(const int* par, int l, int r0, int c0, int RW, int gy) {
    while (true) {
        const int me = (r0 + l / RW) * gy + (c0 + l % RW);
        const int p = par[l];
        if (p == me) return l;
        l = (p / gy - r0) * RW + (p % gy - c0);
    }
}

__global__ __launch_bounds__(kUfThreads) void dbscan_union_tiled_kernel(Cfg c, const uint8_t* __restrict__ dyn,
                                                                        const uint8_t* __restrict__ core, const float* __restrict__ xs,
                                                                        const float* __restrict__ ys, const float* __restrict__ flow,
                                                                        int* __restrict__ parent, int tiles_r, int tiles_c) {
    __shared__ int s_par[kRegMax];
    __shared__ float s_f[kRegMax][3];
    __shared__ uint8_t s_core[kRegMax];
    __shared__ int s_any;
    const int b = blockIdx.y;
    const int tr = blockIdx.x / tiles_c, tc = blockIdx.x % tiles_c;
    const int tid = threadIdx.x;
    const size_t per = (size_t)c.gx * c.gy, base = (size_t)b * per;
    if (tid == 0) s_any = 0;
    __syncthreads();
    int any = 0;
    for (int q = tid; q < kTR * kTC; q += kUfThreads) {
        const int r = tr * kTR + q / kTC, col = tc * kTC + q % kTC;
        if (r < c.gx && col < c.gy && core[base + (size_t)r * c.gy + col]) any = 1;
    }
    if (any) s_any = 1;
    __syncthreads();
    if (!s_any) return;
    const int r0 = max(tr * kTR - c.win, 0), r1 = min(tr * kTR + kTR + c.win, c.gx);
    const int c0 = max(tc * kTC - c.win, 0), c1 = min(tc * kTC + kTC + c.win, c.gy);
    const int RW = c1 - c0, RH = r1 - r0, RN = RW * RH;
    for (int l = tid; l < RN; l += kUfThreads) {
        const int r = r0 + l / RW, col = c0 + l % RW;
        const size_t g = base + (size_t)r * c.gy + col;
        const uint8_t co = core[g];
        s_core[l] = co;
        s_par[l] = r * c.gy + col;
        if (co) {
            s_f[l][0] = c.flow_weight * flow[3 * g + 0];
            s_f[l][1] = c.flow_weight * flow[3 * g + 1];
            s_f[l][2] = c.flow_weight * flow[3 * g + 2];
        }
    }
    __syncthreads();
    __shared__ int s_list[kTR * kTC];
    __shared__ int s_n;
    if (tid == 0) s_n = 0;
    __syncthreads();
    for (int q = tid; q < kTR * kTC; q += kUfThreads) {
        const int r = tr * kTR + q / kTC, col = tc * kTC + q % kTC;
        if (r < c.gx && col < c.gy && s_core[(r - r0) * RW + (col - c0)]) s_list[atomicAdd(&s_n, 1)] = q;
    }
    __syncthreads();
    const int n_list = s_n, lane = tid & 63, wave = tid >> 6;
    const int ww = 2 * c.win + 1;
    for (int e = wave; e < n_list; e += kUfThreads / 64) {
        const int q = s_list[e];
        const int r = tr * kTR + q / kTC, col = tc * kTC + q % kTC;
        const int lx = (r - r0) * RW + (col - c0);
        const double x0 = (double)xs[r], y0 = (double)ys[col];
        const double f0 = (double)s_f[lx][0], f1 = (double)s_f[lx][1], f2 = (double)s_f[lx][2];
        const int n_win = c.win * ww + c.win;
        for (int k = lane; k < n_win; k += 64) {
            const int rr = r - c.win + k / ww, cc = col - c.win + k % ww;
            if (rr < 0 || cc < 0 || cc >= c.gy) continue;
            const int ly = (rr - r0) * RW + (cc - c0);
            if (!s_core[ly]) continue;
            const double d0 = x0 - (double)xs[rr], d1 = y0 - (double)ys[cc];
            const double d2 = f0 - (double)s_f[ly][0], d3 = f1 - (double)s_f[ly][1], d4 = f2 - (double)s_f[ly][2];
            if (d0 * d0 + d1 * d1 + d2 * d2 + d3 * d3 + d4 * d4 > c.eps_sqr) continue;
            int a = lx, bq = ly;
            while (true) {
                a = lds_find(s_par, a, r0, c0, RW, c.gy);
                bq = lds_find(s_par, bq, r0, c0, RW, c.gy);
                if (a == bq) break;
                const int ga = (r0 + a / RW) * c.gy + (c0 + a % RW), gb = (r0 + bq / RW) * c.gy + (c0 + bq % RW);
                int hi = a, lo_g = gb, hi_g = ga;
                if (ga < gb) { hi = bq; lo_g = ga; hi_g = gb; }
                const int old = atomicMin(&s_par[hi], lo_g);
                if (old == hi_g) break;
                a = (old / c.gy - r0) * RW + (old % c.gy - c0);
                bq = (lo_g / c.gy - r0) * RW + (lo_g % c.gy - c0);
            }
        }
    }
    __syncthreads();
    int* par = parent + base;
    for (int l = tid; l < RN; l += kUfThreads) {
        if (!s_core[l]) continue;
        const int me = (r0 + l / RW) * c.gy + (c0 + l % RW);
        const int lr = lds_find(s_par, l, r0, c0, RW, c.gy);
        const int root = (r0 + lr / RW) * c.gy + (c0 + lr % RW);
        if (root == me) continue;
        int x = me, y = root;
        while (true) {
            x = find_root_compress(par, x);
            y = find_root_compress(par, y);
            if (x == y) break;
            if (x < y) { const int t = x; x = y; y = t; }
            const int old = atomicMin(&par[x], y);
            if (old == x) break;
            x = old;
        }
    }
}

__global__ void dbscan_flatten_kernel(Cfg c, const uint8_t* __restrict__ core, int* __restrict__ parent,
                                      int* __restrict__ is_root) {
    const size_t i = (size_t)blockIdx.x * blockDim.x + threadIdx.x;
    const size_t per = (size_t)c.gx * c.gy;
    if (i >= per * c.batch) return;
    int root_flag = 0;
    if (core[i]) {
        const int* par = parent + (i / per) * per;
        const int root = find_root(par, (int)(i % per));
        root_flag = root == (int)(i % per);
    }
    is_root[i] = root_flag;
}

__global__ void dbscan_label_kernel(Cfg c, const uint8_t* __restrict__ dyn, const uint8_t* __restrict__ core,
                                    const float* __restrict__ xs, const float* __restrict__ ys, const float* __restrict__ flow,
                                    const int* __restrict__ parent, const int* __restrict__ root_rank, int* __restrict__ labels) {
    const size_t i = (size_t)blockIdx.x * blockDim.x + threadIdx.x;
    const size_t per = (size_t)c.gx * c.gy;
    if (i >= per * c.batch) return;
    int label = 0;
    if (dyn[i]) {
        const int b = (int)(i / per), r = (int)((i % per) / c.gy), col = (int)(i % c.gy);
        const int* par = parent + (size_t)b * per;
        const int* rank = root_rank + (size_t)b * per;
        if (core[i]) {
            label = rank[find_root(par, (int)(i % per))];
        } else {
            int best = 0x7fffffff;
            for_each_neighbour(c, dyn, xs, ys, flow, b, r, col, [&](size_t nb) {
                if (core[nb]) best = min(best, rank[find_root(par, (int)(nb % per))]);
            });
            label = best == 0x7fffffff ? 0 : best;
        }
    }
    labels[i] = label;
}

__global__ __launch_bounds__(256) void region_moments_kernel(const int* __restrict__ labels, int batch, int gx, int gy, int max_labels,
                                                             unsigned long long* __restrict__ mom) {
    const unsigned i = blockIdx.x * blockDim.x + threadIdx.x;
    const unsigned per = (unsigned)gx * (unsigned)gy;
    const int lane = threadIdx.x & 63;
    int l = i < per * (unsigned)batch ? labels[i] : 0;
    if (l > max_labels) l = 0;
    const unsigned bi = i / per, rem = i - bi * per, ri = rem / (unsigned)gy;
    const long key = l > 0 ? (long)bi * max_labels + (l - 1) : -1;
    const unsigned long long r = ri, col = rem - ri * (unsigned)gy;
    unsigned long long todo = __ballot(key >= 0);
    while (todo) {
        const int src = __ffsll((long long)todo) - 1;
        const long k = __shfl(key, src);
        const bool mine = key == k;
        unsigned long long v[6] = {mine ? 1ull : 0ull, mine ? r : 0ull, mine ? col : 0ull, mine ? r * r : 0ull, mine ? col * col : 0ull,
                                   mine ? r * col : 0ull};
#pragma unroll
        for (int o = 32; o > 0; o >>= 1)
#pragma unroll
            for (int q = 0; q < 6; q++) v[q] += __shfl_xor(v[q], o);
        if (lane == src) {
            unsigned long long* m = mom + (size_t)k * 6;
#pragma unroll
            for (int q = 0; q < 6; q++) atomicAdd(m + q, v[q]);
        }
        todo &= ~__ballot(mine);
    }
}

constexpr int kRmCells = 2048, kRmThreads = 256, kRmMaxLabels = 1024;
__global__ __launch_bounds__(kRmThreads) void region_moments_lds_kernel(const int* __restrict__ labels, int gx, int gy, int max_labels,
                                                                         int blocks_per_sample, unsigned long long* __restrict__ partial) {
    extern __shared__ unsigned long long s_mom[];
    const int b = blockIdx.y, blk = blockIdx.x;
    const unsigned per = (unsigned)gx * (unsigned)gy;
    for (int q = threadIdx.x; q < max_labels * 6; q += kRmThreads) s_mom[q] = 0ull;
    __syncthreads();
    const unsigned c0 = (unsigned)blk * kRmCells;
    for (unsigned c = c0 + threadIdx.x; c < c0 + kRmCells && c < per; c += kRmThreads) {
        int l = labels[(size_t)b * per + c];
        if (l <= 0 || l > max_labels) continue;
        const unsigned long long r = c / (unsigned)gy, col = c - (unsigned)r * (unsigned)gy;
        unsigned long long* m = s_mom + (size_t)(l - 1) * 6;
        atomicAdd(m + 0, 1ull); atomicAdd(m + 1, r); atomicAdd(m + 2, col);
        atomicAdd(m + 3, r * r); atomicAdd(m + 4, col * col); atomicAdd(m + 5, r * col);
    }
    __syncthreads();
    unsigned long long* out = partial + ((size_t)b * blocks_per_sample + blk) * max_labels * 6;
    for (int q = threadIdx.x; q < max_labels * 6; q += kRmThreads) out[q] = s_mom[q];
}

__global__ __launch_bounds__(256) void region_moments_sum_kernel(const unsigned long long* __restrict__ partial, int batch, int max_labels,
                                                                 int blocks_per_sample, unsigned long long* __restrict__ mom) {
    const int region = blockIdx.x * 4 + (threadIdx.x >> 6), lane = threadIdx.x & 63;
    if (region >= batch * max_labels) return;
    const int b = region / max_labels, l = region - b * max_labels;
    unsigned long long v[6] = {0, 0, 0, 0, 0, 0};
    for (int blk = lane; blk < blocks_per_sample; blk += 64) {
        const unsigned long long* p = partial + (((size_t)b * blocks_per_sample + blk) * max_labels + l) * 6;
#pragma unroll
        for (int q = 0; q < 6; q++) v[q] += p[q];
    }
#pragma unroll
    for (int o = 32; o > 0; o >>= 1)
#pragma unroll
        for (int q = 0; q < 6; q++) v[q] += __shfl_xor(v[q], o);
    if (lane < 6) {
        unsigned long long w = v[0];
#pragma unroll
        for (int q = 1; q < 6; q++) w = lane == q ? v[q] : w;
        mom[(size_t)region * 6 + lane] = w;
    }
}

__global__ void region_props_kernel(const unsigned long long* __restrict__ mom, long n_regions, double* __restrict__ props) {
    const long i = (long)blockIdx.x * blockDim.x + threadIdx.x;
    if (i >= n_regions) return;
    const unsigned long long* m = mom + (size_t)i * 6;
    double* p = props + (size_t)i * 5;
    const double n = (double)m[0];
    if (m[0] == 0) { p[0] = p[1] = p[2] = p[3] = p[4] = 0.0; return; }
    const double sr = (double)m[1], sc = (double)m[2];
    const double cr = sr / n, cc = sc / n;
    const double mu20 = ((double)m[3] - sr * sr / n) / n;
    const double mu02 = ((double)m[4] - sc * sc / n) / n;
    const double mu11 = ((double)m[5] - sr * sc / n) / n;
    const double a = mu02, b = -mu11, c = mu20;
    double orientation;
    if (a - c == 0.0)
        orientation = b < 0.0 ? -M_PI / 4.0 : M_PI / 4.0;
    else
        orientation = 0.5 * atan2(-2.0 * b, c - a);
    const double tr = a + c, disc = sqrt((a - c) * (a - c) + 4.0 * b * b);
    const double l1 = fmax(0.5 * (tr + disc), 0.0), l2 = fmax(0.5 * (tr - disc), 0.0);
    p[0] = cr; p[1] = cc; p[2] = orientation; p[3] = 4.0 * sqrt(l1); p[4] = 4.0 * sqrt(l2);
}

inline bool cfg_ok(const liso_dbscan_cfg* c) {
    return c && c->batch >= 1 && c->gx >= 1 && c->gy >= 1 && c->window >= 0 && c->min_samples >= 1 && c->eps > 0.f &&
           (long)c->gx * c->gy < (1L << 31);
}
inline Cfg to_cfg(const liso_dbscan_cfg* c) {
    Cfg k;
    k.batch = c->batch; k.gx = c->gx; k.gy = c->gy; k.win = c->window; k.min_samples = c->min_samples;
    k.eps_sqr = (double)c->eps * (double)c->eps;
    k.flow_weight = c->flow_weight;
    return k;
}

}

extern "C" {

int liso_dbscan_components(const liso_dbscan_cfg* cfg, const uint8_t* dynamic_mask, const float* row_coords,
                           const float* col_coords, const float* flow, uint8_t* core, int32_t* parent, int32_t* is_root,
                           void* stream) {
    if (!cfg_ok(cfg) || !dynamic_mask || !row_coords || !col_coords || !flow || !core || !parent || !is_root) return LISO_EINVAL;
    const Cfg c = to_cfg(cfg);
    const size_t total = (size_t)c.batch * c.gx * c.gy;
    const unsigned blocks = (unsigned)((total + 255) / 256);
    hipStream_t st = (hipStream_t)stream;
    dbscan_core_kernel<<<blocks, 256, 0, st>>>(c, dynamic_mask, row_coords, col_coords, flow, core, parent);
    if (c.win <= kMaxWin) {
        const int tiles_r = (c.gx + kTR - 1) / kTR, tiles_c = (c.gy + kTC - 1) / kTC;
        dbscan_union_tiled_kernel<<<dim3(tiles_r * tiles_c, c.batch), kUfThreads, 0, st>>>(c, dynamic_mask, core, row_coords, col_coords,
                                                                                         flow, parent, tiles_r, tiles_c);
    } else {
        dbscan_union_kernel<<<blocks, 256, 0, st>>>(c, dynamic_mask, core, row_coords, col_coords, flow, parent);
    }
    dbscan_flatten_kernel<<<blocks, 256, 0, st>>>(c, core, parent, is_root);
    return check_launch();
}

int liso_dbscan_labels(const liso_dbscan_cfg* cfg, const uint8_t* dynamic_mask, const float* row_coords, const float* col_coords,
                       const float* flow, const uint8_t* core, const int32_t* parent, const int32_t* root_rank,
                       int32_t* labels, void* stream) {
    if (!cfg_ok(cfg) || !dynamic_mask || !row_coords || !col_coords || !flow || !core || !parent || !root_rank || !labels)
        return LISO_EINVAL;
    const Cfg c = to_cfg(cfg);
    const size_t total = (size_t)c.batch * c.gx * c.gy;
    dbscan_label_kernel<<<(unsigned)((total + 255) / 256), 256, 0, (hipStream_t)stream>>>(c, dynamic_mask, core, row_coords,
                                                                                       col_coords, flow, parent, root_rank, labels);
    return check_launch();
}

int liso_region_props(const int32_t* labels, int batch, int gx, int gy, int max_labels, uint64_t* moments, double* props,
                      void* stream) {
    if (!labels || batch < 1 || gx < 1 || gy < 1 || max_labels < 1 || !moments || !props) return LISO_EINVAL;
    if ((size_t)batch * gx * gy >= (1ull << 31)) return LISO_EINVAL;
    hipStream_t st = (hipStream_t)stream;
    const size_t total = (size_t)batch * gx * gy;
    const long regions = (long)batch * max_labels;
    if (liso_zero::zero_async(moments, (size_t)regions * 6 * sizeof(uint64_t), st) != hipSuccess) return LISO_ELAUNCH;
    region_moments_kernel<<<(unsigned)((total + 255) / 256), 256, 0, st>>>(labels, batch, gx, gy, max_labels,
                                                                          (unsigned long long*)moments);
    region_props_kernel<<<(unsigned)((regions + 255) / 256), 256, 0, st>>>((const unsigned long long*)moments, regions, props);
    return check_launch();
}

size_t liso_region_props_workspace_bytes(int batch, int gx, int gy, int max_labels) {
    if (batch < 1 || gx < 1 || gy < 1 || max_labels < 1 || max_labels > kRmMaxLabels) return 0;
    const size_t per = (size_t)gx * gy;
    if (per * batch >= (1ull << 31)) return 0;
    const size_t blocks = (per + kRmCells - 1) / kRmCells;
    return (size_t)batch * blocks * max_labels * 6 * sizeof(uint64_t);
}

int liso_region_props_ws(const int32_t* labels, int batch, int gx, int gy, int max_labels, uint64_t* moments, double* props,
                         void* workspace, size_t workspace_bytes, void* stream) {
    if (!labels || batch < 1 || gx < 1 || gy < 1 || max_labels < 1 || !moments || !props) return LISO_EINVAL;
    const size_t need = liso_region_props_workspace_bytes(batch, gx, gy, max_labels);
    if (need == 0) return liso_region_props(labels, batch, gx, gy, max_labels, moments, props, stream);
    if (!workspace || workspace_bytes < need) return LISO_EWORKSPACE;
    hipStream_t st = (hipStream_t)stream;
    const int blocks = (int)(((size_t)gx * gy + kRmCells - 1) / kRmCells);
    const long regions = (long)batch * max_labels;
    region_moments_lds_kernel<<<dim3(blocks, batch), kRmThreads, (size_t)max_labels * 6 * sizeof(uint64_t), st>>>(
        labels, gx, gy, max_labels, blocks, (unsigned long long*)workspace);
    region_moments_sum_kernel<<<(unsigned)((regions + 3) / 4), 256, 0, st>>>((const unsigned long long*)workspace, batch, max_labels,
                                                                            blocks, (unsigned long long*)moments);
    region_props_kernel<<<(unsigned)((regions + 255) / 256), 256, 0, st>>>((const unsigned long long*)moments, regions, props);
    return check_launch();
}

}
```

liso_amd/networks/flow_cluster_detector/flow_cluster_detector.py:

```python
import numpy as np
import torch

from liso_amd import _lib as L
from liso_amd.kabsch.shape_utils import Shape, extract_motion_in_pred_box_coordinates
from liso_amd.utils.bev_flow_utils import get_bev_dynamic_flow_map_from_pcl_flow_and_odom


@torch.no_grad()
def fit_bev_box_z_and_height_using_points_in_box(pcl, boxes: Shape, box_height=1000.0):
    assert len(pcl.shape) == 2, pcl.shape
    assert len(boxes.pos.shape) == 2, boxes.pos.shape
    L.require_cuda(pcl)
    dev = pcl.device
    pts = pcl.float().contiguous()
    K = boxes.pos.shape[0]
    num = torch.zeros(K, dtype=torch.int64, device=dev)
    fz = torch.zeros(K, dtype=torch.float32, device=dev)
    fh = torch.zeros(K, dtype=torch.float32, device=dev)
    if K == 0:
        return num, fz, fh
    pos, dims, rot = boxes.pos.float().contiguous(), boxes.dims.float().contiguous(), boxes.rot[..., 0].float().contiguous()
    lib = L.lib()
    nbytes = lib.liso_fit_box_z_workspace_bytes(pts.shape[0], K)
    ws = torch.empty(max(nbytes, 8), dtype=torch.uint8, device=dev)
    with torch.cuda.device(dev):
        L.check(L.TIMER.launch("fit_box_z", lambda: lib.liso_fit_box_z_f32(
            L.ptr(pts), pts.shape[-1], pts.shape[0], L.ptr(pos), pos.shape[-1], L.ptr(dims), dims.shape[-1], L.ptr(rot), K,
            float(box_height), L.ptr(num), L.ptr(fz), L.ptr(fh), L.ptr(ws), nbytes, L.stream_ptr())), "fit_box_z")
    return num, fz, fh


@torch.no_grad()
def cluster_dynamic_pillars(dynamic_mask, bev_nonrigid_flow, row_coords_m, col_coords_m, eps=1.0, min_samples=5,
                            flow_similarity_importance=2.0, pitch=None):
    L.require_cuda(dynamic_mask, bev_nonrigid_flow)
    B, gx, gy = dynamic_mask.shape
    dev = dynamic_mask.device
    dyn = dynamic_mask.to(torch.uint8).contiguous()
    flow = bev_nonrigid_flow.float().contiguous()
    assert flow.shape == (B, gx, gy, 3), flow.shape
    xs, ys = row_coords_m.float().contiguous(), col_coords_m.float().contiguous()
    if pitch is None:
        pitch = min(float(xs[1] - xs[0]) if gx > 1 else eps, float(ys[1] - ys[0]) if gy > 1 else eps)
    cfg = L.DbscanCfg(B, gx, gy, int(eps / pitch) + 1, int(min_samples), float(eps), float(flow_similarity_importance))
    core = torch.empty((B, gx, gy), dtype=torch.uint8, device=dev)
    parent = torch.empty((B, gx, gy), dtype=torch.int32, device=dev)
    is_root = torch.empty((B, gx, gy), dtype=torch.int32, device=dev)
    labels = torch.empty((B, gx, gy), dtype=torch.int32, device=dev)
    lib = L.lib()
    import ctypes
    with torch.cuda.device(dev):
        L.check(L.TIMER.launch("dbscan_components", lambda: lib.liso_dbscan_components(
            ctypes.byref(cfg), L.ptr(dyn), L.ptr(xs), L.ptr(ys), L.ptr(flow), L.ptr(core), L.ptr(parent), L.ptr(is_root),
            L.stream_ptr())), "dbscan_components")
        from liso_amd.networks.flow_cluster_detector.mining_ops import inclusive_scan_i32
        rank = inclusive_scan_i32(is_root.view(B, -1)).view(B, gx, gy)
        L.check(L.TIMER.launch("dbscan_labels", lambda: lib.liso_dbscan_labels(
            ctypes.byref(cfg), L.ptr(dyn), L.ptr(xs), L.ptr(ys), L.ptr(flow), L.ptr(core), L.ptr(parent), L.ptr(rank),
            L.ptr(labels), L.stream_ptr())), "dbscan_labels")
    return labels, rank.view(B, -1)[:, -1].long()


@torch.no_grad()
def label_region_props(labels, max_labels):
    L.require_cuda(labels)
    B, gx, gy = labels.shape
    lab = labels.to(torch.int32).contiguous()
    mom = torch.empty((B, max_labels, 6), dtype=torch.int64, device=lab.device)
    props = torch.empty((B, max_labels, 5), dtype=torch.float64, device=lab.device)
    lib = L.lib()
    nbytes = lib.liso_region_props_workspace_bytes(B, gx, gy, max_labels)
    ws = torch.empty(max(nbytes, 8), dtype=torch.uint8, device=lab.device)
    with torch.cuda.device(lab.device):
        L.check(L.TIMER.launch("region_props", lambda: lib.liso_region_props_ws(
            L.ptr(lab), B, gx, gy, max_labels, L.ptr(mom), L.ptr(props), L.ptr(ws), nbytes, L.stream_ptr())), "region_props")
    return props


class FlowClusterDetector(torch.nn.Module):

    def __init__(self, cfg, min_num_pts_per_box=10, max_box_len_m=7.0, aspect_ratio_max=4.0, min_box_area_m2=0.35,
                 min_box_volume_m3=0.5) -> None:
        super().__init__()
        from liso_amd.kabsch.kabsch_mask import KabschDecoder
        from liso_amd.utils.bev_utils import get_bev_setup_params

        tcfg = cfg.data.tracking_cfg
        if getattr(tcfg, "flow_cluster_detector_ignore_min_box_size_limits", False):
            min_box_area_m2, min_box_volume_m3 = 0.0, 0.0
        if getattr(tcfg, "flow_cluster_detector_ignore_max_box_size_limits", False):
            aspect_ratio_max, max_box_len_m = 1000.0, 1000.0
        self.min_box_area_m2, self.min_box_volume_m3 = min_box_area_m2, min_box_volume_m3
        self.min_num_pts_per_box, self.aspect_ratio_max, self.max_box_len_m = min_num_pts_per_box, aspect_ratio_max, max_box_len_m
        self.cfg = cfg
        (self.bev_range_m_np, self.img_grid_size_np, self.bev_pixel_per_meter_res_np, self.pcl_bev_center_coords_homog_np,
         torch_params) = get_bev_setup_params(cfg)
        for name, param in torch_params.items():
            self.register_parameter(name, torch.nn.Parameter(param, requires_grad=False))
        self.min_residual_flow_thresh_mps = 1.0
        self.bev_img_grid_size = np.array(self.cfg.data.img_grid_size)
        self.kabsch_decoder = KabschDecoder(cfg)
        c = self.pcl_bev_center_coords_homog_np
        dx = float(np.float32(c[1, 0, 0]) - np.float32(c[0, 0, 0])) if c.shape[0] > 1 else 1.0
        dy = float(np.float32(c[0, 1, 1]) - np.float32(c[0, 0, 1])) if c.shape[1] > 1 else 1.0
        self._pitch = min(dx, dy)
        self.last_num_labels = None
        self.register_buffer("_row_coords", torch.from_numpy(np.ascontiguousarray(c[:, 0, 0])).float(), persistent=False)
        self.register_buffer("_col_coords", torch.from_numpy(np.ascontiguousarray(c[0, :, 1])).float(), persistent=False)

    @torch.no_grad()
    def forward(self, sample_data_ta, writer=None, writer_prefix: str = "", global_step: int = None, is_batched=True,
                capacity: int = None, odom_minus_eye=None) -> Shape:
        pcl = sample_data_ta["pcl_ta"]["pcl"]
        pcl_w_ground = sample_data_ta["pcl_full_w_ground_ta"]
        pillar_coors = sample_data_ta["pcl_ta"]["pillar_coors"]
        point_flow = sample_data_ta[self.cfg.data.flow_source]["flow_ta_tb"]
        odom_ta_tb = sample_data_ta[self.cfg.data.odom_source]["odom_ta_tb"]
        thresh = sample_data_ta["src_trgt_time_delta_s"] * self.min_residual_flow_thresh_mps
        if is_batched:
            pcl_is_valid = sample_data_ta["pcl_ta"]["pcl_is_valid"]
        else:
            pcl_is_valid = torch.ones_like(pcl[:, 0], dtype=torch.bool)[None]
            pcl, pcl_w_ground, pillar_coors = pcl[None], pcl_w_ground[None], pillar_coors[None]
            point_flow, odom_ta_tb, thresh = point_flow[None], odom_ta_tb[None], thresh[None]
        dev = pcl.device
        bev_dynamicness, bev_nonrigid_flow = get_bev_dynamic_flow_map_from_pcl_flow_and_odom(
            pcl_is_valid=pcl_is_valid, pcl=pcl, pillar_coors=pillar_coors, point_flow=point_flow, odom_ta_tb=odom_ta_tb,
            target_shape=self.bev_img_grid_size, return_nonrigid_bev_flow=True, odom_minus_eye=odom_minus_eye)
        dynamic_mask = torch.squeeze(bev_dynamicness, dim=-1) > thresh.to(dev)[..., None, None]
        centers = self.pcl_bev_center_coords_homog
        labels, num_labels = cluster_dynamic_pillars(dynamic_mask, bev_nonrigid_flow, self._row_coords, self._col_coords,
                                                     pitch=self._pitch if capacity else None)
        self.last_bev_labels, self.last_num_labels = labels, num_labels
        B = labels.shape[0]
        if capacity:
            k_max = int(capacity)
        else:
            k_max = int(num_labels.max()) if B > 0 else 0
        if k_max == 0:
            boxes = Shape.from_list_of_shapes([Shape.createEmpty().to_tensor().to(dev) for _ in range(B)], numeric_padding_value=0.0)
            return boxes if is_batched else boxes[0]
        props = label_region_props(labels, k_max)
        from liso_amd.kabsch.shape_utils import Shape as _Shape
        from liso_amd.networks.flow_cluster_detector import mining_ops as MO

        ppm = self.bev_pixel_per_meter_res_np
        center, dims2, rot1, dims2_f32, rot1_f32 = MO.boxes_from_regions(props, self._row_coords, self._col_coords, ppm)
        assert dims2.shape[-1] == 2, "otherwise box fitting will use bad box size from clustering!"
        zbuf = torch.zeros(B * k_max * 16, dtype=torch.uint8, device=dev)
        num_pts = zbuf[:B * k_max * 8].view(torch.int64).view(B, k_max)
        fit_z = zbuf[B * k_max * 8:B * k_max * 12].view(torch.float32).view(B, k_max)
        fit_h = zbuf[B * k_max * 12:].view(torch.float32).view(B, k_max)
        lib = L.lib()
        for b in range(B):
            pts = pcl_w_ground[b].float().contiguous()
            nbytes = lib.liso_fit_box_z_workspace_bytes(pts.shape[0], k_max)
            ws = torch.empty(max(nbytes, 8), dtype=torch.uint8, device=dev)
            with torch.cuda.device(dev):
                L.check(L.TIMER.launch("fit_box_z", lambda: lib.liso_fit_box_z_f32(
                    L.ptr(pts), pts.shape[-1], pts.shape[0], L.ptr(center[b]), 2, L.ptr(dims2_f32[b]), 2, L.ptr(rot1_f32[b]), k_max,
                    1000.0, L.ptr(num_pts[b]), L.ptr(fit_z[b]), L.ptr(fit_h[b]), L.ptr(ws), nbytes, L.stream_ptr())), "fit_box_z")
        arr = MO.filter_compact(num_labels, center, dims2, rot1, num_pts, fit_z, fit_h, min_points=self.min_num_pts_per_box,
                                aspect_ratio_max=self.aspect_ratio_max, max_box_len_m=self.max_box_len_m,
                                min_box_area_m2=self.min_box_area_m2, min_box_volume_m3=self.min_box_volume_m3,
                                park_invalid=bool(capacity))
        s_max = k_max if capacity else int(arr["counts"].max())

        def cut(t):
            return t if s_max == t.shape[1] else t[:, :s_max].contiguous()

        keep = cut(arr["valid"]).view(torch.bool)
        boxes = _Shape(pos=cut(arr["pos"]), dims=cut(arr["dims"]), rot=cut(arr["rot"]), probs=cut(arr["probs"]), velo=cut(arr["velo"]),
                       valid=keep, class_id=cut(arr["class_id"]), difficulty=cut(arr["difficulty"]))
        if s_max > 0:
            kboxes = _Shape(pos=cut(arr["kabsch_pos"]), dims=cut(arr["kabsch_dims"]), rot=cut(arr["kabsch_rot"])[..., None],
                            probs=boxes.probs, valid=keep)
            trafos = self.kabsch_decoder.trafos_from_point_flow_packed(
                point_cloud_ta=pcl, valid_mask_ta=pcl_is_valid, pointwise_flow_ta_tb=point_flow, pred_boxes_ta=kboxes,
                slot_count=arr["counts"] if capacity else None)
            MO.box_motion(trafos, boxes.pos, boxes.rot, boxes.velo)
        if not is_batched:
            boxes = boxes[0]
            assert len(boxes.shape) == 1, boxes.shape
        return boxes
```

liso_amd/networks/flow_cluster_detector/mining_ops.py:

```python
import ctypes

import torch

from liso_amd import _lib as L


def inclusive_scan_i32(x):
    L.require_cuda(x)
    assert x.dtype == torch.int32 and x.dim() == 2 and x.is_contiguous()
    B, n = x.shape
    out = torch.empty_like(x)
    lib = L.lib()
    nbytes = lib.liso_scan_workspace_bytes(B, n)
    ws = torch.empty(max(nbytes, 8), dtype=torch.uint8, device=x.device)
    with torch.cuda.device(x.device):
        L.check(lib.liso_scan_inclusive_i32(L.ptr(x), B, n, L.ptr(out), L.ptr(ws), nbytes, L.stream_ptr()), "scan_inclusive_i32")
    return out


def boxes_from_regions(props, row_coords, col_coords, ppm):
    L.require_cuda(props)
    B, K, _ = props.shape
    dev = props.device
    props = props.contiguous()
    center = torch.empty((B, K, 2), dtype=torch.float32, device=dev)
    dims = torch.empty((B, K, 2), dtype=torch.float64, device=dev)
    rot = torch.empty((B, K), dtype=torch.float64, device=dev)
    dims32 = torch.empty((B, K, 2), dtype=torch.float32, device=dev)
    rot32 = torch.empty((B, K), dtype=torch.float32, device=dev)
    with torch.cuda.device(dev):
        L.check(L.lib().liso_mine_boxes_from_regions(
            L.ptr(props), B, K, L.ptr(row_coords), row_coords.shape[0], L.ptr(col_coords), col_coords.shape[0], float(ppm[0]),
            float(ppm[1]), L.ptr(center), L.ptr(dims), L.ptr(rot), L.ptr(dims32), L.ptr(rot32), L.stream_ptr()), "mine_boxes_from_regions")
    return center, dims, rot, dims32, rot32


def filter_compact(num_labels, center, dims2, rot, num_pts, fit_z, fit_h, *, min_points, aspect_ratio_max, max_box_len_m,
                   min_box_area_m2, min_box_volume_m3, park_invalid):
    B, K, _ = center.shape
    dev = center.device
    f32, f64, i32 = torch.float32, torch.float64, torch.int32
    o = {"pos": torch.empty((B, K, 3), dtype=f32, device=dev), "dims": torch.empty((B, K, 3), dtype=f64, device=dev),
         "rot": torch.empty((B, K, 1), dtype=f64, device=dev), "probs": torch.empty((B, K, 1), dtype=f64, device=dev),
         "velo": torch.empty((B, K, 1), dtype=f64, device=dev), "valid": torch.empty((B, K), dtype=torch.uint8, device=dev),
         "class_id": torch.empty((B, K, 1), dtype=i32, device=dev), "difficulty": torch.empty((B, K, 1), dtype=i32, device=dev),
         "counts": torch.empty((B,), dtype=i32, device=dev), "kabsch_pos": torch.empty((B, K, 3), dtype=f32, device=dev),
         "kabsch_dims": torch.empty((B, K, 3), dtype=f32, device=dev), "kabsch_rot": torch.empty((B, K), dtype=f32, device=dev)}
    cfg = L.MineFilterCfg(B, K, int(min_points), float(aspect_ratio_max), float(max_box_len_m), float(min_box_area_m2),
                          float(min_box_volume_m3), int(bool(park_invalid)))
    nl = num_labels.to(torch.int64).contiguous()
    with torch.cuda.device(dev):
        L.check(L.lib().liso_mine_filter_compact(
            ctypes.byref(cfg), L.ptr(nl), L.ptr(center), L.ptr(dims2), L.ptr(rot), L.ptr(num_pts), L.ptr(fit_z), L.ptr(fit_h),
            L.ptr(o["pos"]), L.ptr(o["dims"]), L.ptr(o["rot"]), L.ptr(o["probs"]), L.ptr(o["velo"]), L.ptr(o["valid"]),
            L.ptr(o["class_id"]), L.ptr(o["difficulty"]), L.ptr(o["counts"]), L.ptr(o["kabsch_pos"]), L.ptr(o["kabsch_dims"]),
            L.ptr(o["kabsch_rot"]), L.stream_ptr()), "mine_filter_compact")
    return o


def box_motion(trafos, pos, rot, velo):
    B, S1 = trafos.shape[:2]
    S = S1 - 1
    assert pos.shape == (B, S, 3) and pos.dtype == torch.float32 and pos.is_contiguous()
    assert rot.shape == (B, S, 1) and rot.dtype == torch.float64 and rot.is_contiguous() and velo.is_contiguous()
    assert trafos.dtype == torch.float64 and trafos.is_contiguous()
    with torch.cuda.device(pos.device):
        L.check(L.lib().liso_mine_box_motion(L.ptr(trafos), B, S, L.ptr(pos), L.ptr(rot), L.ptr(velo), L.stream_ptr()), "mine_box_motion")


def nms_select(arrays, max_num_boxes, overlap_threshold, pre_nms_max_num_boxes, targets_out=None):
    from liso_amd import iou3d_nms_cuda

    pos = arrays["pos"]
    B, K, _ = pos.shape
    dev = pos.device
    lib = L.lib()
    dense = torch.empty((B, K, 7), dtype=torch.float32, device=dev)
    enters = torch.empty((B, K), dtype=torch.uint8, device=dev)
    nbytes = lib.liso_mine_nms_workspace_bytes(B, K)
    ws = torch.empty(nbytes, dtype=torch.uint8, device=dev)
    a = arrays
    with torch.cuda.device(dev):
        L.check(lib.liso_mine_nms_prepare(
            B, K, int(pre_nms_max_num_boxes), L.ptr(a["pos"]), L.ptr(a["dims"]), L.ptr(a["rot"]), L.ptr(a["probs"]), L.ptr(a["velo"]),
            L.ptr(a["valid"]), L.ptr(a["class_id"]), L.ptr(a["difficulty"]), L.ptr(dense), L.ptr(enters), L.ptr(ws), nbytes,
            L.stream_ptr()), "mine_nms_prepare")
    if targets_out is None:
        targets_out = (torch.empty((B, K, 3), dtype=torch.float32, device=dev), torch.empty((B, K, 3), dtype=torch.float32, device=dev),
                       torch.empty((B, K), dtype=torch.float32, device=dev), torch.empty((B, K), dtype=torch.uint8, device=dev))
    t_pos, t_dims, t_rot, t_valid = targets_out
    for b in range(B):
        keep_dev, num_dev = iou3d_nms_cuda.nms_gpu_device(dense[b], overlap_threshold)
        with torch.cuda.device(dev):
            L.check(lib.liso_mine_nms_finish(
                b, K, int(max_num_boxes), L.ptr(keep_dev), L.ptr(num_dev), L.ptr(enters), L.ptr(a["pos"]), L.ptr(a["dims"]),
                L.ptr(a["rot"]), L.ptr(a["probs"]), L.ptr(a["velo"]), L.ptr(a["valid"]), L.ptr(a["class_id"]), L.ptr(a["difficulty"]),
                L.ptr(t_pos), L.ptr(t_dims), L.ptr(t_rot), L.ptr(t_valid), L.stream_ptr()), "mine_nms_finish")
    return t_pos, t_dims, t_rot, t_valid
```

liso_amd/utils/bev_flow_utils.py:

```python
import torch

from liso_amd import _lib as L


@torch.no_grad()
def get_bev_dynamic_flow_map_from_pcl_flow_and_odom(*, pcl_is_valid, pcl, pillar_coors, point_flow, odom_ta_tb,
                                                    target_shape, return_nonrigid_bev_flow=False, odom_minus_eye=None):
    L.require_cuda(pcl, point_flow)
    B, N = pcl_is_valid.shape
    h, w = int(target_shape[0]), int(target_shape[1])
    dev = pcl.device
    pts = pcl.float().contiguous()
    fl = point_flow.float().contiguous()
    assert fl.shape[-1] >= 3, fl.shape
    val = pcl_is_valid.to(torch.uint8).contiguous()
    coors = pillar_coors.to(torch.int32).contiguous()
    ome = odom_minus_eye if odom_minus_eye is not None else odometry_minus_identity(odom_ta_tb)
    dyn = torch.empty((B, h, w, 1), dtype=torch.float32, device=dev)
    nrf = torch.empty((B, h, w, 3), dtype=torch.float32, device=dev)
    lib = L.lib()
    nbytes = lib.liso_bev_dynamic_flow_workspace_bytes(B, h, w)
    ws = torch.empty(nbytes, dtype=torch.uint8, device=dev)
    with torch.cuda.device(dev):
        L.check(L.TIMER.launch("bev_dynamic_flow", lambda: lib.liso_bev_dynamic_flow_f32(
            L.ptr(pts), pts.shape[-1], L.ptr(val), L.ptr(coors), L.ptr(fl), fl.shape[-1], L.ptr(ome), B, N, h, w,
            L.ptr(dyn), L.ptr(nrf), L.ptr(ws), nbytes, L.stream_ptr())), "bev_dynamic_flow")
    if return_nonrigid_bev_flow:
        return dyn, nrf
    return dyn


@torch.no_grad()
def odometry_minus_identity(odom_ta_tb):
    dev = odom_ta_tb.device
    if not odom_ta_tb.is_cuda:
        return (torch.linalg.inv_ex(odom_ta_tb.double()).inverse - torch.eye(4, device=dev, dtype=torch.float64)[None]).contiguous()
    m = odom_ta_tb.double().contiguous()
    out = torch.empty_like(m)
    with torch.cuda.device(dev):
        L.check(L.lib().liso_odom_inverse_minus_eye_f64(L.ptr(m), m.numel() // 16, L.ptr(out), L.stream_ptr()), "odom_inverse_minus_eye")
    return out
```

Baseline: 1016.

## Fuse box-mining stages: dynamic mask, region boxes, batched fit-z with filter-compact

Folds the dynamic-threshold mask into the BEV mean kernel, fuses region props with box-from-region conversion, and batches fit-z across samples via blockIdx.z. A new fit-final-filter kernel does the per-box reduction and compaction in one launch per sample. This removes several kernel launches, per-sample Python loops and intermediate round trips, and avoids a host sync on num_labels. The cost is a larger block (1024 threads) with shared arrays sized for K up to 2048, plus a fallback path for larger K.

```diff
diff --git a/include/liso_box_mining.h b/include/liso_box_mining.h
--- a/include/liso_box_mining.h
+++ b/include/liso_box_mining.h
@@ -32,6 +32,13 @@
                              int32_t* difficulty, int32_t* counts, float* kabsch_pos, float* kabsch_dims, float* kabsch_rot,
                              void* stream);
 
+int liso_mine_fit_z_filter_compact(const liso_mine_filter_cfg* cfg, const float* points, int point_stride, int n, float box_height,
+                                   const int32_t* num_labels, long num_labels_stride, const float* center, const double* dims2,
+                                   const double* rot_in, const float* dims2_f32, const float* rot_f32, int64_t* num_pts, float* fit_z,
+                                   float* fit_h, float* pos, double* dims, double* rot, double* probs, double* velo, uint8_t* valid,
+                                   int32_t* class_id, int32_t* difficulty, int32_t* counts, float* kabsch_pos, float* kabsch_dims,
+                                   float* kabsch_rot, void* workspace, size_t workspace_bytes, void* stream);
+
 int liso_mine_box_motion(const double* trafos, int batch, int s, const float* pos, double* rot, double* velo, void* stream);
 
 size_t liso_mine_nms_workspace_bytes(int batch, int k);
diff --git a/include/liso_flow_cluster.h b/include/liso_flow_cluster.h
--- a/include/liso_flow_cluster.h
+++ b/include/liso_flow_cluster.h
@@ -14,6 +14,11 @@
                               const float* flow, int flow_stride, const double* odom_minus_eye, int batch, int n, int h,
                               int w, float* dynamicness, float* nonrigid_flow, void* workspace, size_t workspace_bytes,
                               void* stream);
+
+int liso_bev_dynamic_mask_f32(const float* points, int point_stride, const uint8_t* valid, const int32_t* pillar_coors,
+                              const float* flow, int flow_stride, const double* odom_minus_eye, int batch, int n, int h,
+                              int w, const void* thresh, int thresh_is_f64, double thresh_scale, float* dynamicness,
+                              float* nonrigid_flow, uint8_t* dynamic_mask, void* workspace, size_t workspace_bytes, void* stream);
 
 int liso_odom_inverse_minus_eye_f64(const double* odom, int batch, double* out, void* stream);
 
@@ -47,6 +52,10 @@
 int liso_region_props_ws(const int32_t* labels, int batch, int gx, int gy, int max_labels, uint64_t* moments, double* props,
                          void* workspace, size_t workspace_bytes, void* stream);
 
+int liso_region_boxes_ws(const int32_t* labels, int batch, int gx, int gy, int max_labels, uint64_t* moments, double* props,
+                         const float* row_coords, const float* col_coords, float ppm_x, float ppm_y, float* center, double* dims,
+                         double* rot, float* dims_f32, float* rot_f32, void* workspace, size_t workspace_bytes, void* stream);
+
 #ifdef __cplusplus
 }
 #endif
diff --git a/liso_amd/_lib.py b/liso_amd/_lib.py
--- a/liso_amd/_lib.py
+++ b/liso_amd/_lib.py
@@ -138,6 +138,7 @@
     "liso_weighted_moments_bwd_f32": (_i, [_vp, _vp, _vp, _i, ctypes.c_long, _vp, _vp, _vp, _vp, _vp]),
     "liso_bev_dynamic_flow_workspace_bytes": (_sz, [_i, _i, _i]),
     "liso_bev_dynamic_flow_f32": (_i, [_vp, _i, _vp, _vp, _vp, _i, _vp, _i, _i, _i, _i, _vp, _vp, _vp, _sz, _vp]),
+    "liso_bev_dynamic_mask_f32": (_i, [_vp, _i, _vp, _vp, _vp, _i, _vp, _i, _i, _i, _i, _vp, _i, ctypes.c_double, _vp, _vp, _vp, _vp, _sz, _vp]),
     "liso_odom_inverse_minus_eye_f64": (_i, [_vp, _i, _vp, _vp]),
     "liso_fit_box_z_workspace_bytes": (_sz, [_i, _i]),
     "liso_fit_box_z_f32": (_i, [_vp, _i, _i, _vp, _i, _vp, _i, _vp, _i, _f, _vp, _vp, _vp, _vp, _sz, _vp]),
@@ -146,6 +147,7 @@
     "liso_region_props": (_i, [_vp, _i, _i, _i, _i, _vp, _vp, _vp]),
     "liso_region_props_workspace_bytes": (_sz, [_i, _i, _i, _i]),
     "liso_region_props_ws": (_i, [_vp, _i, _i, _i, _i, _vp, _vp, _vp, _sz, _vp]),
+    "liso_region_boxes_ws": (_i, [_vp, _i, _i, _i, _i, _vp, _vp, _vp, _vp, _f, _f, _vp, _vp, _vp, _vp, _vp, _vp, _sz, _vp]),
     "liso_corr_lookup_fwd_f32": (_i, [_vp, _vp, _vp, _vp, _vp, _vp]),
     "liso_corr_lookup_fwd_tiled_f32": (_i, [_vp, _vp, _vp, _vp, _vp, _vp]),
     "liso_corr_lookup_bwd_dvol_f32": (_i, [_vp, _vp, _vp, _vp, _vp]),
@@ -201,6 +203,7 @@
     "liso_scan_inclusive_i32": (_i, [_vp, _i, ctypes.c_long, _vp, _vp, _sz, _vp]),
     "liso_mine_boxes_from_regions": (_i, [_vp, _i, _i, _vp, _i, _vp, _i, _f, _f, _vp, _vp, _vp, _vp, _vp, _vp]),
     "liso_mine_filter_compact": (_i, [_vp] * 21),
+    "liso_mine_fit_z_filter_compact": (_i, [_vp, _vp, _i, _i, _f, _vp, ctypes.c_long] + [_vp] * 21 + [_sz, _vp]),
     "liso_mine_box_motion": (_i, [_vp, _i, _i, _vp, _vp, _vp, _vp]),
     "liso_mine_nms_workspace_bytes": (_sz, [_i, _i]),
     "liso_mine_nms_prepare": (_i, [_i, _i, _i] + [_vp] * 11 + [_sz, _vp]),
diff --git a/liso_amd/csrc/box_mining.hip b/liso_amd/csrc/box_mining.hip
--- a/liso_amd/csrc/box_mining.hip
+++ b/liso_amd/csrc/box_mining.hip
@@ -5,16 +5,17 @@
 #include "../../include/liso_box_mining.h"
 #include "../../include/liso_iou3d.h"
 #include "dev_common.h"
+#include "mine_bodies.h"
 
 namespace {
 
 using liso_dev::check_launch;
+using liso_mine::kInvalidClass;
+using liso_mine::kUnknownClass;
 
 constexpr int kScanThreads = 256;
 constexpr int kScanPer = 8;
 constexpr int kScanChunk = kScanThreads * kScanPer;
-constexpr int32_t kUnknownClass = 2147483647;
-constexpr int32_t kInvalidClass = kUnknownClass - 1;
 
 __device__ __forceinline__ int block_exclusive_scan(int v, int* total) {
     __shared__ int wsum[kScanThreads / 64];
@@ -90,20 +91,7 @@
                                           float* __restrict__ dims_f32, float* __restrict__ rot_f32) {
     const long i = (long)blockIdx.x * blockDim.x + threadIdx.x;
     if (i >= total) return;
-    const double* p = props + i * 5;
-    const long hi = (gx < gy ? gx : gy) - 1;
-    long r = (long)p[0], c = (long)p[1];
-    r = r < 0 ? 0 : (r > hi ? hi : r);
-    c = c < 0 ? 0 : (c > hi ? hi : c);
-    center[i * 2 + 0] = row_coords[r];
-    center[i * 2 + 1] = col_coords[c];
-    const double d0 = p[3] * 1.0 / ppm_x, d1 = p[4] * 1.0 / ppm_y;
-    dims[i * 2 + 0] = d0;
-    dims[i * 2 + 1] = d1;
-    rot[i] = p[2];
-    dims_f32[i * 2 + 0] = (float)d0;
-    dims_f32[i * 2 + 1] = (float)d1;
-    rot_f32[i] = (float)p[2];
+    liso_mine::boxes_from_regions_body(props + i * 5, i, row_coords, gx, col_coords, gy, ppm_x, ppm_y, center, dims, rot, dims_f32, rot_f32);
 }
 
 __global__ __launch_bounds__(64) void filter_compact_kernel(const liso_mine_filter_cfg c, const int64_t* __restrict__ num_labels,
@@ -115,64 +103,11 @@
                                                             uint8_t* __restrict__ valid, int32_t* __restrict__ class_id,
                                                             int32_t* __restrict__ difficulty, int32_t* __restrict__ counts,
                                                             float* __restrict__ kpos, float* __restrict__ kdims, float* __restrict__ krot) {
-    const int b = blockIdx.x, lane = threadIdx.x, K = c.k;
-    const long o = (long)b * K;
-    const long nl = num_labels[b];
-    int run = 0;
-    for (int k0 = 0; k0 < K; k0 += 64) {
-        const int k = k0 + lane;
-        bool ok = false;
-        double d0 = 0.0, d1 = 0.0, hz = 0.0, th = 0.0;
-        float cx = 0.f, cy = 0.f, fz = 0.f;
-        if (k < K) {
-            d0 = dims2[(o + k) * 2];
-            d1 = dims2[(o + k) * 2 + 1];
-            hz = (double)fit_h[o + k];
-            th = rot_in[o + k];
-            cx = center[(o + k) * 2];
-            cy = center[(o + k) * 2 + 1];
-            fz = fit_z[o + k];
-            const bool exists = k < nl;
-            const bool enough = num_pts[o + k] >= (int64_t)c.min_points;
-            const double aspect = d0 / fmax(d1, 0.001);
-            const bool aspect_ok = aspect <= c.aspect_ratio_max;
-            const bool not_large = d0 <= c.max_box_len_m;
-            const bool foot_ok = d0 * d1 > c.min_box_area_m2;
-            const bool vol_ok = (d0 * d1) * hz > c.min_box_volume_m3;
-            ok = exists && enough && aspect_ok && not_large && foot_ok && vol_ok;
-        }
-        const unsigned long long m = __ballot(ok);
-        const int dst = run + __popcll(m & ((1ull << lane) - 1ull));
-        if (ok) {
-            const long q = o + dst;
-            pos[q * 3] = cx, pos[q * 3 + 1] = cy, pos[q * 3 + 2] = fz;
-            dims[q * 3] = d0, dims[q * 3 + 1] = d1, dims[q * 3 + 2] = hz;
-            rot[q] = th;
-            probs[q] = 1.0;
-            velo[q] = 0.0;
-            valid[q] = 1;
-            class_id[q] = kUnknownClass;
-            difficulty[q] = 1;
-            kpos[q * 3] = cx, kpos[q * 3 + 1] = cy, kpos[q * 3 + 2] = fz;
-            kdims[q * 3] = (float)d0, kdims[q * 3 + 1] = (float)d1, kdims[q * 3 + 2] = (float)hz;
-            krot[q] = (float)th;
-        }
-        run += __popcll(m);
-    }
-    for (int k = run + lane; k < K; k += 64) {
-        const long q = o + k;
-        pos[q * 3] = 0.f, pos[q * 3 + 1] = 0.f, pos[q * 3 + 2] = 0.f;
-        dims[q * 3] = 0.0, dims[q * 3 + 1] = 0.0, dims[q * 3 + 2] = 0.0;
-        rot[q] = 0.0, probs[q] = 0.0, velo[q] = 0.0;
-        valid[q] = 0;
-        class_id[q] = kInvalidClass;
-        difficulty[q] = kInvalidClass;
-        const float park = c.park_invalid ? 1e6f : 0.f;
-        kpos[q * 3] = park, kpos[q * 3 + 1] = park, kpos[q * 3 + 2] = park;
-        kdims[q * 3] = 0.f, kdims[q * 3 + 1] = 0.f, kdims[q * 3 + 2] = 0.f;
-        krot[q] = 0.f;
-    }
-    if (lane == 0) counts[b] = run;
+    const int b = blockIdx.x;
+    const long o = (long)b * c.k;
+    liso_mine::filter_compact_body(c, threadIdx.x, num_labels[b], center + o * 2, dims2 + o * 2, rot_in + o, (const long long*)num_pts + o,
+                                   fit_z + o, fit_h + o, pos + o * 3, dims + o * 3, rot + o, probs + o, velo + o, valid + o, class_id + o,
+                                   difficulty + o, counts + b, kpos + o * 3, kdims + o * 3, krot + o);
 }
 
 struct Aff {
diff --git a/liso_amd/csrc/flow_cluster.hip b/liso_amd/csrc/flow_cluster.hip
--- a/liso_amd/csrc/flow_cluster.hip
+++ b/liso_amd/csrc/flow_cluster.hip
@@ -6,6 +6,7 @@
 #include "../../include/liso_flow_cluster.h"
 #include "../../include/liso_iou3d.h"
 #include "dev_common.h"
+#include "mine_bodies.h"
 
 namespace {
 
@@ -70,7 +71,8 @@
 }
 
 __global__ void bev_mean_kernel(const long long* __restrict__ sums, const int* __restrict__ counts, size_t cells,
-                                float* __restrict__ dyn, float* __restrict__ nrflow) {
+                                float* __restrict__ dyn, float* __restrict__ nrflow, const void* __restrict__ thresh, int thresh_f64,
+                                double thresh_scale, size_t cells_per_sample, uint8_t* __restrict__ mask) {
     const size_t i = (size_t)blockIdx.x * blockDim.x + threadIdx.x;
     if (i >= cells) return;
     const int cnt = counts[i];
@@ -82,6 +84,11 @@
     }
     dyn[i] = v[0];
     nrflow[i * 3 + 0] = v[1]; nrflow[i * 3 + 1] = v[2]; nrflow[i * 3 + 2] = v[3];
+    if (mask) {
+        const size_t b = i / cells_per_sample;
+        const double t = thresh_f64 ? ((const double*)thresh)[b] * thresh_scale : (double)(((const float*)thresh)[b] * (float)thresh_scale);
+        mask[i] = (double)v[0] > t ? 1 : 0;
+    }
 }
 
 constexpr int kFitThreads = 256;
@@ -98,8 +105,14 @@
                                                             const float* __restrict__ box_pos, int pos_dims,
                                                             const float* __restrict__ box_dims, int dims_dims,
                                                             const float* __restrict__ box_rot, int k, float box_height,
-                                                            FitPartial* __restrict__ partials, int tiles_per_block) {
+                                                            FitPartial* __restrict__ partials, int tiles_per_block,
+                                                            size_t sample_stride) {
     __shared__ float px[kFitTile], py[kFitTile], pz[kFitTile];
+    points += blockIdx.z * sample_stride;
+    box_pos += (size_t)blockIdx.z * k * pos_dims;
+    box_dims += (size_t)blockIdx.z * k * dims_dims;
+    box_rot += (size_t)blockIdx.z * k;
+    partials += (size_t)blockIdx.z * gridDim.x * k;
     __shared__ FitPartial red[kFitThreads / 64][64];
     const int tid = threadIdx.x, lane = tid & 63, wave = tid >> 6;
     const int box = blockIdx.y * 64 + lane;
@@ -153,12 +166,13 @@
     }
 }
 
-__global__ __launch_bounds__(64) void fit_z_final_kernel(const FitPartial* __restrict__ partials, int nblk, int k,
-                                                         const float* __restrict__ points, int ps, int n, float box_height,
-                                                         long long* __restrict__ num_pts, float* __restrict__ fz,
-                                                         float* __restrict__ fh) {
-    const int box = blockIdx.x, lane = threadIdx.x;
-    if (box >= k) return;
+struct FitResult {
+    long long num;
+    float z, height;
+};
+
+__device__ __forceinline__ FitResult fit_z_final_body(const FitPartial* __restrict__ partials, int nblk, int k, int box, int lane,
+                                                      const float* __restrict__ points, int n, float box_height) {
     FitPartial r = {0, box_height, -box_height, 0.f, 0x7fffffff};
     for (int b = lane; b < nblk; b += 64) {
         const FitPartial o = partials[(size_t)b * k + box];
@@ -178,12 +192,59 @@
         r.zmax = fmaxf(r.zmax, o.zmax);
         if (o.zmin < r.zmin || (o.zmin == r.zmin && o.zmin_idx < r.zmin_idx)) { r.zmin = o.zmin; r.zmin_sensor = o.zmin_sensor; r.zmin_idx = o.zmin_idx; }
     }
-    if (lane != 0) return;
     const float height = fminf(fmaxf(r.zmax - r.zmin, 1.0f), 2.0f);
     const float zlow = r.count > 0 ? r.zmin_sensor : (n > 0 ? points[2] : 0.f);
-    num_pts[box] = r.count;
-    fh[box] = height;
-    fz[box] = zlow + 0.5f * height;
+    FitResult f;
+    f.num = r.count;
+    f.height = height;
+    f.z = zlow + 0.5f * height;
+    return f;
+}
+
+__global__ __launch_bounds__(64) void fit_z_final_kernel(const FitPartial* __restrict__ partials, int nblk, int k,
+                                                         const float* __restrict__ points, int ps, int n, float box_height,
+                                                         long long* __restrict__ num_pts, float* __restrict__ fz,
+                                                         float* __restrict__ fh) {
+    const int box = blockIdx.x, lane = threadIdx.x;
+    if (box >= k) return;
+    const FitResult f = fit_z_final_body(partials, nblk, k, box, lane, points, n, box_height);
+    if (lane != 0) return;
+    num_pts[box] = f.num;
+    fh[box] = f.height;
+    fz[box] = f.z;
+}
+
+constexpr int kFitFilterMaxK = 2048, kFitFilterThreads = 1024;
+__global__ __launch_bounds__(kFitFilterThreads) void fit_final_filter_kernel(const FitPartial* __restrict__ partials, int nblk,
+                                                               const float* __restrict__ points, size_t sample_stride, int n,
+                                                               float box_height, const liso_mine_filter_cfg c,
+                                                               const int32_t* __restrict__ num_labels, long num_labels_stride,
+                                                               const float* __restrict__ center, const double* __restrict__ dims2,
+                                                               const double* __restrict__ rot_in, long long* __restrict__ num_pts,
+                                                               float* __restrict__ fit_z, float* __restrict__ fit_h,
+                                                               float* __restrict__ pos, double* __restrict__ dims, double* __restrict__ rot,
+                                                               double* __restrict__ probs, double* __restrict__ velo,
+                                                               uint8_t* __restrict__ valid, int32_t* __restrict__ class_id,
+                                                               int32_t* __restrict__ difficulty, int32_t* __restrict__ counts,
+                                                               float* __restrict__ kpos, float* __restrict__ kdims, float* __restrict__ krot) {
+    __shared__ long long s_num[kFitFilterMaxK];
+    __shared__ float s_z[kFitFilterMaxK], s_h[kFitFilterMaxK];
+    const int b = blockIdx.x, lane = threadIdx.x & 63, wave = threadIdx.x >> 6, K = c.k;
+    const long o = (long)b * K;
+    const FitPartial* pb = partials + (size_t)b * nblk * K;
+    const float* pts = points + b * sample_stride;
+    for (int box = wave; box < K; box += kFitFilterThreads / 64) {
+        const FitResult f = fit_z_final_body(pb, nblk, K, box, lane, pts, n, box_height);
+        if (lane == 0) {
+            num_pts[o + box] = f.num, fit_h[o + box] = f.height, fit_z[o + box] = f.z;
+            s_num[box] = f.num, s_h[box] = f.height, s_z[box] = f.z;
+        }
+    }
+    __syncthreads();
+    if (wave != 0) return;
+    liso_mine::filter_compact_body(c, lane, (long)num_labels[b * num_labels_stride], center + o * 2, dims2 + o * 2, rot_in + o, s_num, s_z, s_h,
+                                   pos + o * 3, dims + o * 3, rot + o, probs + o, velo + o, valid + o, class_id + o, difficulty + o,
+                                   counts + b, kpos + o * 3, kdims + o * 3, krot + o);
 }
 
 __global__ void odom_inverse_minus_eye_kernel(const double* __restrict__ m_all, int batch, double* __restrict__ out_all) {
@@ -230,10 +291,14 @@
     return (size_t)batch * h * w * (4 * sizeof(long long) + sizeof(int));
 }
 
-int liso_bev_dynamic_flow_f32(const float* points, int point_stride, const uint8_t* valid, const int32_t* pillar_coors,
-                              const float* flow, int flow_stride, const double* odom_minus_eye, int batch, int n, int h,
-                              int w, float* dynamicness, float* nonrigid_flow, void* workspace, size_t workspace_bytes,
-                              void* stream) {
+}
+
+namespace {
+
+int bev_dynamic_flow(const float* points, int point_stride, const uint8_t* valid, const int32_t* pillar_coors, const float* flow,
+                     int flow_stride, const double* odom_minus_eye, int batch, int n, int h, int w, float* dynamicness,
+                     float* nonrigid_flow, const void* thresh, int thresh_is_f64, double thresh_scale, uint8_t* dynamic_mask,
+                     void* workspace, size_t workspace_bytes, void* stream) {
     if (batch <= 0 || n < 0 || h <= 0 || w <= 0 || point_stride < 3 || flow_stride < 3) return LISO_EINVAL;
     if (!dynamicness || !nonrigid_flow || !workspace || !odom_minus_eye) return LISO_EINVAL;
     if (n > 0 && (!points || !valid || !pillar_coors || !flow)) return LISO_EINVAL;
@@ -249,8 +314,30 @@
         bev_scatter_kernel<<<(unsigned)((total + 255) / 256), 256, 0, st>>>(points, point_stride, valid, pillar_coors, flow,
                                                                           flow_stride, odom_minus_eye, batch, n, h, w, sums,
                                                                           counts);
-    bev_mean_kernel<<<(unsigned)((cells + 255) / 256), 256, 0, st>>>(sums, counts, cells, dynamicness, nonrigid_flow);
+    bev_mean_kernel<<<(unsigned)((cells + 255) / 256), 256, 0, st>>>(sums, counts, cells, dynamicness, nonrigid_flow, thresh, thresh_is_f64,
+                                                                     thresh_scale, (size_t)h * w, dynamic_mask);
     return check_launch();
+}
+
+}
+
+extern "C" {
+
+int liso_bev_dynamic_flow_f32(const float* points, int point_stride, const uint8_t* valid, const int32_t* pillar_coors,
+                              const float* flow, int flow_stride, const double* odom_minus_eye, int batch, int n, int h,
+                              int w, float* dynamicness, float* nonrigid_flow, void* workspace, size_t workspace_bytes,
+                              void* stream) {
+    return bev_dynamic_flow(points, point_stride, valid, pillar_coors, flow, flow_stride, odom_minus_eye, batch, n, h, w, dynamicness,
+                            nonrigid_flow, nullptr, 0, 0.0, nullptr, workspace, workspace_bytes, stream);
+}
+
+int liso_bev_dynamic_mask_f32(const float* points, int point_stride, const uint8_t* valid, const int32_t* pillar_coors,
+                              const float* flow, int flow_stride, const double* odom_minus_eye, int batch, int n, int h,
+                              int w, const void* thresh, int thresh_is_f64, double thresh_scale, float* dynamicness,
+                              float* nonrigid_flow, uint8_t* dynamic_mask, void* workspace, size_t workspace_bytes, void* stream) {
+    if (!thresh || !dynamic_mask) return LISO_EINVAL;
+    return bev_dynamic_flow(points, point_stride, valid, pillar_coors, flow, flow_stride, odom_minus_eye, batch, n, h, w, dynamicness,
+                            nonrigid_flow, thresh, thresh_is_f64, thresh_scale, dynamic_mask, workspace, workspace_bytes, stream);
 }
 
 int liso_odom_inverse_minus_eye_f64(const double* odom, int batch, double* out, void* stream) {
@@ -281,10 +368,37 @@
     const int tpb = (tiles + nblk - 1) / nblk > 0 ? (tiles + nblk - 1) / nblk : 1;
     fit_z_kernel<<<dim3(nblk, (k + 63) / 64), kFitThreads, 0, st>>>(points, point_stride, n, box_pos, pos_dims, box_dims,
                                                                     dims_dims, box_rot, k, box_height,
-                                                                    (FitPartial*)workspace, tpb);
+                                                                    (FitPartial*)workspace, tpb, 0);
     fit_z_final_kernel<<<k, 64, 0, st>>>((const FitPartial*)workspace, nblk, k, points, point_stride, n,
                                                      box_height, (long long*)num_pts, fitted_z, fitted_height);
     return check_launch();
 }
 
-}
+int liso_mine_fit_z_filter_compact(const liso_mine_filter_cfg* cfg, const float* points, int point_stride, int n, float box_height,
+                                   const int32_t* num_labels, long num_labels_stride, const float* center, const double* dims2,
+                                   const double* rot_in, const float* dims2_f32, const float* rot_f32, int64_t* num_pts, float* fit_z,
+                                   float* fit_h, float* pos, double* dims, double* rot, double* probs, double* velo, uint8_t* valid,
+                                   int32_t* class_id, int32_t* difficulty, int32_t* counts, float* kabsch_pos, float* kabsch_dims,
+                                   float* kabsch_rot, void* workspace, size_t workspace_bytes, void* stream) {
+    if (!cfg || cfg->batch <= 0 || cfg->k <= 0 || cfg->k > kFitFilterMaxK || n < 0 || point_stride < 3 || num_labels_stride < 0)
+        return LISO_EINVAL;
+    if (!num_labels || !center || !dims2 || !rot_in || !dims2_f32 || !rot_f32 || !num_pts || !fit_z || !fit_h || !pos || !dims || !rot ||
+        !probs || !velo || !valid || !class_id || !difficulty || !counts || !kabsch_pos || !kabsch_dims || !kabsch_rot || !workspace ||
+        (n > 0 && !points))
+        return LISO_EINVAL;
+    if (workspace_bytes < (size_t)cfg->batch * liso_fit_box_z_workspace_bytes(n, cfg->k)) return LISO_EWORKSPACE;
+    hipStream_t st = (hipStream_t)stream;
+    const int k = cfg->k, nblk = fit_blocks(n);
+    const int tiles = (n + kFitTile - 1) / kFitTile;
+    const int tpb = (tiles + nblk - 1) / nblk > 0 ? (tiles + nblk - 1) / nblk : 1;
+    const size_t sample_stride = (size_t)n * point_stride;
+    fit_z_kernel<<<dim3(nblk, (k + 63) / 64, cfg->batch), kFitThreads, 0, st>>>(points, point_stride, n, center, 2, dims2_f32, 2, rot_f32, k,
+                                                                                box_height, (FitPartial*)workspace, tpb, sample_stride);
+    fit_final_filter_kernel<<<cfg->batch, kFitFilterThreads, 0, st>>>((const FitPartial*)workspace, nblk, points, sample_stride, n, box_height, *cfg,
+                                                        num_labels, num_labels_stride, center, dims2, rot_in, (long long*)num_pts, fit_z,
+                                                        fit_h, pos, dims, rot, probs, velo, valid, class_id, difficulty, counts, kabsch_pos,
+                                                        kabsch_dims, kabsch_rot);
+    return check_launch();
+}
+
+}
diff --git a/liso_amd/csrc/flow_dbscan.hip b/liso_amd/csrc/flow_dbscan.hip
--- a/liso_amd/csrc/flow_dbscan.hip
+++ b/liso_amd/csrc/flow_dbscan.hip
@@ -7,6 +7,7 @@
 #include "../../include/liso_flow_cluster.h"
 #include "../../include/liso_iou3d.h"
 #include "dev_common.h"
+#include "mine_bodies.h"
 
 namespace {
 
@@ -389,24 +390,36 @@
 __global__ void region_props_kernel(const unsigned long long* __restrict__ mom, long n_regions, double* __restrict__ props) {
     const long i = (long)blockIdx.x * blockDim.x + threadIdx.x;
     if (i >= n_regions) return;
-    const unsigned long long* m = mom + (size_t)i * 6;
-    double* p = props + (size_t)i * 5;
-    const double n = (double)m[0];
-    if (m[0] == 0) { p[0] = p[1] = p[2] = p[3] = p[4] = 0.0; return; }
-    const double sr = (double)m[1], sc = (double)m[2];
-    const double cr = sr / n, cc = sc / n;
-    const double mu20 = ((double)m[3] - sr * sr / n) / n;
-    const double mu02 = ((double)m[4] - sc * sc / n) / n;
-    const double mu11 = ((double)m[5] - sr * sc / n) / n;
-    const double a = mu02, b = -mu11, c = mu20;
-    double orientation;
-    if (a - c == 0.0)
-        orientation = b < 0.0 ? -M_PI / 4.0 : M_PI / 4.0;
-    else
-        orientation = 0.5 * atan2(-2.0 * b, c - a);
-    const double tr = a + c, disc = sqrt((a - c) * (a - c) + 4.0 * b * b);
-    const double l1 = fmax(0.5 * (tr + disc), 0.0), l2 = fmax(0.5 * (tr - disc), 0.0);
-    p[0] = cr; p[1] = cc; p[2] = orientation; p[3] = 4.0 * sqrt(l1); p[4] = 4.0 * sqrt(l2);
+    liso_mine::region_props_body(mom + (size_t)i * 6, props + (size_t)i * 5);
+}
+
+__global__ __launch_bounds__(256) void region_boxes_kernel(const unsigned long long* __restrict__ partial, int batch, int max_labels,
+                                                           int blocks_per_sample, unsigned long long* __restrict__ mom,
+                                                           double* __restrict__ props, const float* __restrict__ row_coords, int gx,
+                                                           const float* __restrict__ col_coords, int gy, double ppm_x, double ppm_y,
+                                                           float* __restrict__ center, double* __restrict__ dims, double* __restrict__ rot,
+                                                           float* __restrict__ dims_f32, float* __restrict__ rot_f32) {
+    const int region = blockIdx.x * 4 + (threadIdx.x >> 6), lane = threadIdx.x & 63;
+    if (region >= batch * max_labels) return;
+    const int b = region / max_labels, l = region - b * max_labels;
+    unsigned long long v[6] = {0, 0, 0, 0, 0, 0};
+    for (int blk = lane; blk < blocks_per_sample; blk += 64) {
+        const unsigned long long* p = partial + (((size_t)b * blocks_per_sample + blk) * max_labels + l) * 6;
+#pragma unroll
+        for (int q = 0; q < 6; q++) v[q] += p[q];
+    }
+#pragma unroll
+    for (int o = 32; o > 0; o >>= 1)
+#pragma unroll
+        for (int q = 0; q < 6; q++) v[q] += __shfl_xor(v[q], o);
+    if (lane != 0) return;
+    double p[5];
+    liso_mine::region_props_body(v, p);
+#pragma unroll
+    for (int q = 0; q < 6; q++) mom[(size_t)region * 6 + q] = v[q];
+#pragma unroll
+    for (int q = 0; q < 5; q++) props[(size_t)region * 5 + q] = p[q];
+    liso_mine::boxes_from_regions_body(p, region, row_coords, gx, col_coords, gy, ppm_x, ppm_y, center, dims, rot, dims_f32, rot_f32);
 }
 
 inline bool cfg_ok(const liso_dbscan_cfg* c) {
@@ -496,4 +509,23 @@
     return check_launch();
 }
 
-}
+int liso_region_boxes_ws(const int32_t* labels, int batch, int gx, int gy, int max_labels, uint64_t* moments, double* props,
+                         const float* row_coords, const float* col_coords, float ppm_x, float ppm_y, float* center, double* dims,
+                         double* rot, float* dims_f32, float* rot_f32, void* workspace, size_t workspace_bytes, void* stream) {
+    if (!labels || batch < 1 || gx < 1 || gy < 1 || max_labels < 1 || !moments || !props) return LISO_EINVAL;
+    if (!row_coords || !col_coords || !center || !dims || !rot || !dims_f32 || !rot_f32) return LISO_EINVAL;
+    const size_t need = liso_region_props_workspace_bytes(batch, gx, gy, max_labels);
+    if (need == 0) return LISO_EINVAL;
+    if (!workspace || workspace_bytes < need) return LISO_EWORKSPACE;
+    hipStream_t st = (hipStream_t)stream;
+    const int blocks = (int)(((size_t)gx * gy + kRmCells - 1) / kRmCells);
+    const long regions = (long)batch * max_labels;
+    region_moments_lds_kernel<<<dim3(blocks, batch), kRmThreads, (size_t)max_labels * 6 * sizeof(uint64_t), st>>>(
+        labels, gx, gy, max_labels, blocks, (unsigned long long*)workspace);
+    region_boxes_kernel<<<(unsigned)((regions + 3) / 4), 256, 0, st>>>(
+        (const unsigned long long*)workspace, batch, max_labels, blocks, (unsigned long long*)moments, props, row_coords, gx, col_coords, gy,
+        (double)ppm_x, (double)ppm_y, center, dims, rot, dims_f32, rot_f32);
+    return check_launch();
+}
+
+}
diff --git a/liso_amd/csrc/mine_bodies.h b/liso_amd/csrc/mine_bodies.h
--- /dev/null
+++ b/liso_amd/csrc/mine_bodies.h
@@ -0,0 +1,114 @@
+#pragma once
+#include <hip/hip_runtime.h>
+#include <math.h>
+#include <stdint.h>
+
+#include "../../include/liso_box_mining.h"
+
+namespace liso_mine {
+
+constexpr int32_t kUnknownClass = 2147483647;
+constexpr int32_t kInvalidClass = kUnknownClass - 1;
+
+__device__ __forceinline__ void region_props_body(const unsigned long long* m, double* p) {
+    const double n = (double)m[0];
+    if (m[0] == 0) { p[0] = p[1] = p[2] = p[3] = p[4] = 0.0; return; }
+    const double sr = (double)m[1], sc = (double)m[2];
+    const double cr = sr / n, cc = sc / n;
+    const double mu20 = ((double)m[3] - sr * sr / n) / n;
+    const double mu02 = ((double)m[4] - sc * sc / n) / n;
+    const double mu11 = ((double)m[5] - sr * sc / n) / n;
+    const double a = mu02, b = -mu11, c = mu20;
+    double orientation;
+    if (a - c == 0.0)
+        orientation = b < 0.0 ? -M_PI / 4.0 : M_PI / 4.0;
+    else
+        orientation = 0.5 * atan2(-2.0 * b, c - a);
+    const double tr = a + c, disc = sqrt((a - c) * (a - c) + 4.0 * b * b);
+    const double l1 = fmax(0.5 * (tr + disc), 0.0), l2 = fmax(0.5 * (tr - disc), 0.0);
+    p[0] = cr; p[1] = cc; p[2] = orientation; p[3] = 4.0 * sqrt(l1); p[4] = 4.0 * sqrt(l2);
+}
+
+__device__ __forceinline__ void boxes_from_regions_body(const double* p, long i, const float* __restrict__ row_coords, int gx,
+                                                        const float* __restrict__ col_coords, int gy, double ppm_x, double ppm_y,
+                                                        float* __restrict__ center, double* __restrict__ dims, double* __restrict__ rot,
+                                                        float* __restrict__ dims_f32, float* __restrict__ rot_f32) {
+    const long hi = (gx < gy ? gx : gy) - 1;
+    long r = (long)p[0], c = (long)p[1];
+    r = r < 0 ? 0 : (r > hi ? hi : r);
+    c = c < 0 ? 0 : (c > hi ? hi : c);
+    center[i * 2 + 0] = row_coords[r];
+    center[i * 2 + 1] = col_coords[c];
+    const double d0 = p[3] * 1.0 / ppm_x, d1 = p[4] * 1.0 / ppm_y;
+    dims[i * 2 + 0] = d0;
+    dims[i * 2 + 1] = d1;
+    rot[i] = p[2];
+    dims_f32[i * 2 + 0] = (float)d0;
+    dims_f32[i * 2 + 1] = (float)d1;
+    rot_f32[i] = (float)p[2];
+}
+
+__device__ __forceinline__ void filter_compact_body(const liso_mine_filter_cfg& c, int lane, long nl, const float* center,
+                                                    const double* dims2, const double* rot_in, const long long* num_pts,
+                                                    const float* fit_z, const float* fit_h, float* pos, double* dims, double* rot,
+                                                    double* probs, double* velo, uint8_t* valid, int32_t* class_id, int32_t* difficulty,
+                                                    int32_t* count, float* kpos, float* kdims, float* krot) {
+    const int K = c.k;
+    int run = 0;
+    for (int k0 = 0; k0 < K; k0 += 64) {
+        const int k = k0 + lane;
+        bool ok = false;
+        double d0 = 0.0, d1 = 0.0, hz = 0.0, th = 0.0;
+        float cx = 0.f, cy = 0.f, fz = 0.f;
+        if (k < K) {
+            d0 = dims2[k * 2];
+            d1 = dims2[k * 2 + 1];
+            hz = (double)fit_h[k];
+            th = rot_in[k];
+            cx = center[k * 2];
+            cy = center[k * 2 + 1];
+            fz = fit_z[k];
+            const bool exists = k < nl;
+            const bool enough = num_pts[k] >= (long long)c.min_points;
+            const double aspect = d0 / fmax(d1, 0.001);
+            const bool aspect_ok = aspect <= c.aspect_ratio_max;
+            const bool not_large = d0 <= c.max_box_len_m;
+            const bool foot_ok = d0 * d1 > c.min_box_area_m2;
+            const bool vol_ok = (d0 * d1) * hz > c.min_box_volume_m3;
+            ok = exists && enough && aspect_ok && not_large && foot_ok && vol_ok;
+        }
+        const unsigned long long m = __ballot(ok);
+        const int dst = run + __popcll(m & ((1ull << lane) - 1ull));
+        if (ok) {
+            const long q = dst;
+            pos[q * 3] = cx, pos[q * 3 + 1] = cy, pos[q * 3 + 2] = fz;
+            dims[q * 3] = d0, dims[q * 3 + 1] = d1, dims[q * 3 + 2] = hz;
+            rot[q] = th;
+            probs[q] = 1.0;
+            velo[q] = 0.0;
+            valid[q] = 1;
+            class_id[q] = kUnknownClass;
+            difficulty[q] = 1;
+            kpos[q * 3] = cx, kpos[q * 3 + 1] = cy, kpos[q * 3 + 2] = fz;
+            kdims[q * 3] = (float)d0, kdims[q * 3 + 1] = (float)d1, kdims[q * 3 + 2] = (float)hz;
+            krot[q] = (float)th;
+        }
+        run += __popcll(m);
+    }
+    for (int k = run + lane; k < K; k += 64) {
+        const long q = k;
+        pos[q * 3] = 0.f, pos[q * 3 + 1] = 0.f, pos[q * 3 + 2] = 0.f;
+        dims[q * 3] = 0.0, dims[q * 3 + 1] = 0.0, dims[q * 3 + 2] = 0.0;
+        rot[q] = 0.0, probs[q] = 0.0, velo[q] = 0.0;
+        valid[q] = 0;
+        class_id[q] = kInvalidClass;
+        difficulty[q] = kInvalidClass;
+        const float park = c.park_invalid ? 1e6f : 0.f;
+        kpos[q * 3] = park, kpos[q * 3 + 1] = park, kpos[q * 3 + 2] = park;
+        kdims[q * 3] = 0.f, kdims[q * 3 + 1] = 0.f, kdims[q * 3 + 2] = 0.f;
+        krot[q] = 0.f;
+    }
+    if (lane == 0) *count = run;
+}
+
+}
diff --git a/liso_amd/networks/flow_cluster_detector/flow_cluster_detector.py b/liso_amd/networks/flow_cluster_detector/flow_cluster_detector.py
--- a/liso_amd/networks/flow_cluster_detector/flow_cluster_detector.py
+++ b/liso_amd/networks/flow_cluster_detector/flow_cluster_detector.py
@@ -32,7 +32,7 @@
 
 @torch.no_grad()
 def cluster_dynamic_pillars(dynamic_mask, bev_nonrigid_flow, row_coords_m, col_coords_m, eps=1.0, min_samples=5,
-                            flow_similarity_importance=2.0, pitch=None):
+                            flow_similarity_importance=2.0, pitch=None, return_rank=False):
     L.require_cuda(dynamic_mask, bev_nonrigid_flow)
     B, gx, gy = dynamic_mask.shape
     dev = dynamic_mask.device
@@ -58,7 +58,8 @@
         L.check(L.TIMER.launch("dbscan_labels", lambda: lib.liso_dbscan_labels(
             ctypes.byref(cfg), L.ptr(dyn), L.ptr(xs), L.ptr(ys), L.ptr(flow), L.ptr(core), L.ptr(parent), L.ptr(rank),
             L.ptr(labels), L.stream_ptr())), "dbscan_labels")
-    return labels, rank.view(B, -1)[:, -1].long()
+    num_labels = rank.view(B, -1)[:, -1].long()
+    return (labels, num_labels, rank.view(B, -1)) if return_rank else (labels, num_labels)
 
 
 @torch.no_grad()
@@ -108,45 +109,11 @@
         self.register_buffer("_row_coords", torch.from_numpy(np.ascontiguousarray(c[:, 0, 0])).float(), persistent=False)
         self.register_buffer("_col_coords", torch.from_numpy(np.ascontiguousarray(c[0, :, 1])).float(), persistent=False)
 
-    @torch.no_grad()
-    def forward(self, sample_data_ta, writer=None, writer_prefix: str = "", global_step: int = None, is_batched=True,
-                capacity: int = None, odom_minus_eye=None) -> Shape:
-        pcl = sample_data_ta["pcl_ta"]["pcl"]
-        pcl_w_ground = sample_data_ta["pcl_full_w_ground_ta"]
-        pillar_coors = sample_data_ta["pcl_ta"]["pillar_coors"]
-        point_flow = sample_data_ta[self.cfg.data.flow_source]["flow_ta_tb"]
-        odom_ta_tb = sample_data_ta[self.cfg.data.odom_source]["odom_ta_tb"]
-        thresh = sample_data_ta["src_trgt_time_delta_s"] * self.min_residual_flow_thresh_mps
-        if is_batched:
-            pcl_is_valid = sample_data_ta["pcl_ta"]["pcl_is_valid"]
-        else:
-            pcl_is_valid = torch.ones_like(pcl[:, 0], dtype=torch.bool)[None]
-            pcl, pcl_w_ground, pillar_coors = pcl[None], pcl_w_ground[None], pillar_coors[None]
-            point_flow, odom_ta_tb, thresh = point_flow[None], odom_ta_tb[None], thresh[None]
-        dev = pcl.device
-        bev_dynamicness, bev_nonrigid_flow = get_bev_dynamic_flow_map_from_pcl_flow_and_odom(
-            pcl_is_valid=pcl_is_valid, pcl=pcl, pillar_coors=pillar_coors, point_flow=point_flow, odom_ta_tb=odom_ta_tb,
-            target_shape=self.bev_img_grid_size, return_nonrigid_bev_flow=True, odom_minus_eye=odom_minus_eye)
-        dynamic_mask = torch.squeeze(bev_dynamicness, dim=-1) > thresh.to(dev)[..., None, None]
-        centers = self.pcl_bev_center_coords_homog
-        labels, num_labels = cluster_dynamic_pillars(dynamic_mask, bev_nonrigid_flow, self._row_coords, self._col_coords,
-                                                     pitch=self._pitch if capacity else None)
-        self.last_bev_labels, self.last_num_labels = labels, num_labels
-        B = labels.shape[0]
-        if capacity:
-            k_max = int(capacity)
-        else:
-            k_max = int(num_labels.max()) if B > 0 else 0
-        if k_max == 0:
-            boxes = Shape.from_list_of_shapes([Shape.createEmpty().to_tensor().to(dev) for _ in range(B)], numeric_padding_value=0.0)
-            return boxes if is_batched else boxes[0]
-        props = label_region_props(labels, k_max)
-        from liso_amd.kabsch.shape_utils import Shape as _Shape
+    def _fit_z_and_filter(self, pcl_w_ground, num_labels, center, dims2, rot1, dims2_f32, rot1_f32, filt):
         from liso_amd.networks.flow_cluster_detector import mining_ops as MO
 
-        ppm = self.bev_pixel_per_meter_res_np
-        center, dims2, rot1, dims2_f32, rot1_f32 = MO.boxes_from_regions(props, self._row_coords, self._col_coords, ppm)
-        assert dims2.shape[-1] == 2, "otherwise box fitting will use bad box size from clustering!"
+        B, k_max = center.shape[:2]
+        dev = center.device
         zbuf = torch.zeros(B * k_max * 16, dtype=torch.uint8, device=dev)
         num_pts = zbuf[:B * k_max * 8].view(torch.int64).view(B, k_max)
         fit_z = zbuf[B * k_max * 8:B * k_max * 12].view(torch.float32).view(B, k_max)
@@ -160,10 +127,69 @@
                 L.check(L.TIMER.launch("fit_box_z", lambda: lib.liso_fit_box_z_f32(
                     L.ptr(pts), pts.shape[-1], pts.shape[0], L.ptr(center[b]), 2, L.ptr(dims2_f32[b]), 2, L.ptr(rot1_f32[b]), k_max,
                     1000.0, L.ptr(num_pts[b]), L.ptr(fit_z[b]), L.ptr(fit_h[b]), L.ptr(ws), nbytes, L.stream_ptr())), "fit_box_z")
-        arr = MO.filter_compact(num_labels, center, dims2, rot1, num_pts, fit_z, fit_h, min_points=self.min_num_pts_per_box,
-                                aspect_ratio_max=self.aspect_ratio_max, max_box_len_m=self.max_box_len_m,
-                                min_box_area_m2=self.min_box_area_m2, min_box_volume_m3=self.min_box_volume_m3,
-                                park_invalid=bool(capacity))
+        return MO.filter_compact(num_labels, center, dims2, rot1, num_pts, fit_z, fit_h, **filt)
+
+    @torch.no_grad()
+    def forward(self, sample_data_ta, writer=None, writer_prefix: str = "", global_step: int = None, is_batched=True,
+                capacity: int = None, odom_minus_eye=None) -> Shape:
+        pcl = sample_data_ta["pcl_ta"]["pcl"]
+        pcl_w_ground = sample_data_ta["pcl_full_w_ground_ta"]
+        pillar_coors = sample_data_ta["pcl_ta"]["pillar_coors"]
+        point_flow = sample_data_ta[self.cfg.data.flow_source]["flow_ta_tb"]
+        odom_ta_tb = sample_data_ta[self.cfg.data.odom_source]["odom_ta_tb"]
+        from liso_amd.networks.flow_cluster_detector import mining_ops as MO
+
+        dt = sample_data_ta["src_trgt_time_delta_s"]
+        fused = bool(capacity) and MO.FUSED
+        fuse_mask = (fused and is_batched and torch.is_tensor(dt) and dt.is_cuda and dt.dim() == 1
+                     and dt.dtype in (torch.float32, torch.float64))
+        thresh = None if fuse_mask else dt * self.min_residual_flow_thresh_mps
+        if is_batched:
+            pcl_is_valid = sample_data_ta["pcl_ta"]["pcl_is_valid"]
+        else:
+            pcl_is_valid = torch.ones_like(pcl[:, 0], dtype=torch.bool)[None]
+            pcl, pcl_w_ground, pillar_coors = pcl[None], pcl_w_ground[None], pillar_coors[None]
+            point_flow, odom_ta_tb, thresh = point_flow[None], odom_ta_tb[None], thresh[None]
+        dev = pcl.device
+        if fuse_mask:
+            bev_dynamicness, bev_nonrigid_flow, dynamic_mask = get_bev_dynamic_flow_map_from_pcl_flow_and_odom(
+                pcl_is_valid=pcl_is_valid, pcl=pcl, pillar_coors=pillar_coors, point_flow=point_flow, odom_ta_tb=odom_ta_tb,
+                target_shape=self.bev_img_grid_size, return_nonrigid_bev_flow=True, odom_minus_eye=odom_minus_eye,
+                dynamic_thresh=dt, dynamic_thresh_scale=self.min_residual_flow_thresh_mps)
+        else:
+            bev_dynamicness, bev_nonrigid_flow = get_bev_dynamic_flow_map_from_pcl_flow_and_odom(
+                pcl_is_valid=pcl_is_valid, pcl=pcl, pillar_coors=pillar_coors, point_flow=point_flow, odom_ta_tb=odom_ta_tb,
+                target_shape=self.bev_img_grid_size, return_nonrigid_bev_flow=True, odom_minus_eye=odom_minus_eye)
+            dynamic_mask = torch.squeeze(bev_dynamicness, dim=-1) > thresh.to(dev)[..., None, None]
+        centers = self.pcl_bev_center_coords_homog
+        labels, num_labels, root_rank = cluster_dynamic_pillars(dynamic_mask, bev_nonrigid_flow, self._row_coords, self._col_coords,
+                                                                pitch=self._pitch if capacity else None, return_rank=True)
+        self.last_bev_labels, self.last_num_labels = labels, num_labels
+        B = labels.shape[0]
+        if capacity:
+            k_max = int(capacity)
+        else:
+            k_max = int(num_labels.max()) if B > 0 else 0
+        if k_max == 0:
+            boxes = Shape.from_list_of_shapes([Shape.createEmpty().to_tensor().to(dev) for _ in range(B)], numeric_padding_value=0.0)
+            return boxes if is_batched else boxes[0]
+        from liso_amd.kabsch.shape_utils import Shape as _Shape
+
+        ppm = self.bev_pixel_per_meter_res_np
+        regions = MO.region_boxes(labels, k_max, self._row_coords, self._col_coords, ppm) if fused else None
+        if regions is not None:
+            center, dims2, rot1, dims2_f32, rot1_f32 = regions[2:]
+        else:
+            props = label_region_props(labels, k_max)
+            center, dims2, rot1, dims2_f32, rot1_f32 = MO.boxes_from_regions(props, self._row_coords, self._col_coords, ppm)
+        assert dims2.shape[-1] == 2, "otherwise box fitting will use bad box size from clustering!"
+        filt = dict(min_points=self.min_num_pts_per_box, aspect_ratio_max=self.aspect_ratio_max, max_box_len_m=self.max_box_len_m,
+                    min_box_area_m2=self.min_box_area_m2, min_box_volume_m3=self.min_box_volume_m3, park_invalid=bool(capacity))
+        if fused and torch.is_tensor(pcl_w_ground) and pcl_w_ground.dim() == 3 and k_max <= 2048:
+            arr = MO.fit_z_filter_compact(pcl_w_ground.float().contiguous(), root_rank, center, dims2, rot1, dims2_f32, rot1_f32,
+                                          box_height=1000.0, **filt)
+        else:
+            arr = self._fit_z_and_filter(pcl_w_ground, num_labels, center, dims2, rot1, dims2_f32, rot1_f32, filt)
         s_max = k_max if capacity else int(arr["counts"].max())
 
         def cut(t):
diff --git a/liso_amd/networks/flow_cluster_detector/mining_ops.py b/liso_amd/networks/flow_cluster_detector/mining_ops.py
--- a/liso_amd/networks/flow_cluster_detector/mining_ops.py
+++ b/liso_amd/networks/flow_cluster_detector/mining_ops.py
@@ -3,6 +3,8 @@
 import torch
 
 from liso_amd import _lib as L
+
+FUSED = True
 
 
 def inclusive_scan_i32(x):
@@ -33,6 +35,66 @@
             L.ptr(props), B, K, L.ptr(row_coords), row_coords.shape[0], L.ptr(col_coords), col_coords.shape[0], float(ppm[0]),
             float(ppm[1]), L.ptr(center), L.ptr(dims), L.ptr(rot), L.ptr(dims32), L.ptr(rot32), L.stream_ptr()), "mine_boxes_from_regions")
     return center, dims, rot, dims32, rot32
+
+
+def region_boxes(labels, max_labels, row_coords, col_coords, ppm):
+    L.require_cuda(labels)
+    B, gx, gy = labels.shape
+    assert labels.dtype == torch.int32 and labels.is_contiguous()
+    assert row_coords.shape[0] == gx and col_coords.shape[0] == gy
+    dev, K, lib = labels.device, int(max_labels), L.lib()
+    nbytes = lib.liso_region_props_workspace_bytes(B, gx, gy, K)
+    if nbytes == 0:
+        return None
+    ws = torch.empty(nbytes, dtype=torch.uint8, device=dev)
+    mom = torch.empty((B, K, 6), dtype=torch.int64, device=dev)
+    props = torch.empty((B, K, 5), dtype=torch.float64, device=dev)
+    center = torch.empty((B, K, 2), dtype=torch.float32, device=dev)
+    dims = torch.empty((B, K, 2), dtype=torch.float64, device=dev)
+    rot = torch.empty((B, K), dtype=torch.float64, device=dev)
+    dims32 = torch.empty((B, K, 2), dtype=torch.float32, device=dev)
+    rot32 = torch.empty((B, K), dtype=torch.float32, device=dev)
+    with torch.cuda.device(dev):
+        L.check(L.TIMER.launch("region_boxes", lambda: lib.liso_region_boxes_ws(
+            L.ptr(labels), B, gx, gy, K, L.ptr(mom), L.ptr(props), L.ptr(row_coords), L.ptr(col_coords), float(ppm[0]), float(ppm[1]),
+            L.ptr(center), L.ptr(dims), L.ptr(rot), L.ptr(dims32), L.ptr(rot32), L.ptr(ws), nbytes, L.stream_ptr())), "region_boxes")
+    return props, mom, center, dims, rot, dims32, rot32
+
+
+def _filter_outputs(B, K, dev):
+    f32, f64, i32 = torch.float32, torch.float64, torch.int32
+    return {"pos": torch.empty((B, K, 3), dtype=f32, device=dev), "dims": torch.empty((B, K, 3), dtype=f64, device=dev),
+            "rot": torch.empty((B, K, 1), dtype=f64, device=dev), "probs": torch.empty((B, K, 1), dtype=f64, device=dev),
+            "velo": torch.empty((B, K, 1), dtype=f64, device=dev), "valid": torch.empty((B, K), dtype=torch.uint8, device=dev),
+            "class_id": torch.empty((B, K, 1), dtype=i32, device=dev), "difficulty": torch.empty((B, K, 1), dtype=i32, device=dev),
+            "counts": torch.empty((B,), dtype=i32, device=dev), "kabsch_pos": torch.empty((B, K, 3), dtype=f32, device=dev),
+            "kabsch_dims": torch.empty((B, K, 3), dtype=f32, device=dev), "kabsch_rot": torch.empty((B, K), dtype=f32, device=dev)}
+
+
+def fit_z_filter_compact(points, root_rank, center, dims2, rot, dims2_f32, rot_f32, *, box_height, min_points, aspect_ratio_max,
+                         max_box_len_m, min_box_area_m2, min_box_volume_m3, park_invalid):
+    L.require_cuda(points)
+    B, K, _ = center.shape
+    dev, lib = center.device, L.lib()
+    assert points.dtype == torch.float32 and points.is_contiguous() and points.shape[0] == B and points.dim() == 3
+    assert root_rank.dtype == torch.int32 and root_rank.is_contiguous() and root_rank.shape[0] == B
+    n = root_rank.shape[1]
+    o = _filter_outputs(B, K, dev)
+    o["num_pts"] = torch.empty((B, K), dtype=torch.int64, device=dev)
+    o["fit_z"] = torch.empty((B, K), dtype=torch.float32, device=dev)
+    o["fit_h"] = torch.empty((B, K), dtype=torch.float32, device=dev)
+    cfg = L.MineFilterCfg(B, K, int(min_points), float(aspect_ratio_max), float(max_box_len_m), float(min_box_area_m2),
+                          float(min_box_volume_m3), int(bool(park_invalid)))
+    nbytes = B * lib.liso_fit_box_z_workspace_bytes(points.shape[1], K)
+    ws = torch.empty(max(nbytes, 8), dtype=torch.uint8, device=dev)
+    with torch.cuda.device(dev):
+        L.check(L.TIMER.launch("fit_z_filter_compact", lambda: lib.liso_mine_fit_z_filter_compact(
+            ctypes.byref(cfg), L.ptr(points), points.shape[-1], points.shape[1], float(box_height), ctypes.c_void_p(root_rank.data_ptr() + 4 * (n - 1)), n,
+            L.ptr(center), L.ptr(dims2), L.ptr(rot), L.ptr(dims2_f32), L.ptr(rot_f32), L.ptr(o["num_pts"]), L.ptr(o["fit_z"]),
+            L.ptr(o["fit_h"]), L.ptr(o["pos"]), L.ptr(o["dims"]), L.ptr(o["rot"]), L.ptr(o["probs"]), L.ptr(o["velo"]), L.ptr(o["valid"]),
+            L.ptr(o["class_id"]), L.ptr(o["difficulty"]), L.ptr(o["counts"]), L.ptr(o["kabsch_pos"]), L.ptr(o["kabsch_dims"]),
+            L.ptr(o["kabsch_rot"]), L.ptr(ws), nbytes, L.stream_ptr())), "fit_z_filter_compact")
+    return o
 
 
 def filter_compact(num_labels, center, dims2, rot, num_pts, fit_z, fit_h, *, min_points, aspect_ratio_max, max_box_len_m,
diff --git a/liso_amd/utils/bev_flow_utils.py b/liso_amd/utils/bev_flow_utils.py
--- a/liso_amd/utils/bev_flow_utils.py
+++ b/liso_amd/utils/bev_flow_utils.py
@@ -5,7 +5,8 @@
 
 @torch.no_grad()
 def get_bev_dynamic_flow_map_from_pcl_flow_and_odom(*, pcl_is_valid, pcl, pillar_coors, point_flow, odom_ta_tb,
-                                                    target_shape, return_nonrigid_bev_flow=False, odom_minus_eye=None):
+                                                    target_shape, return_nonrigid_bev_flow=False, odom_minus_eye=None,
+                                                    dynamic_thresh=None, dynamic_thresh_scale=1.0):
     L.require_cuda(pcl, point_flow)
     B, N = pcl_is_valid.shape
     h, w = int(target_shape[0]), int(target_shape[1])
@@ -21,6 +22,16 @@
     lib = L.lib()
     nbytes = lib.liso_bev_dynamic_flow_workspace_bytes(B, h, w)
     ws = torch.empty(nbytes, dtype=torch.uint8, device=dev)
+    if dynamic_thresh is not None:
+        th = dynamic_thresh.contiguous()
+        assert th.device == dev and th.shape == (B,) and th.dtype in (torch.float32, torch.float64), (th.shape, th.dtype)
+        mask = torch.empty((B, h, w), dtype=torch.uint8, device=dev)
+        with torch.cuda.device(dev):
+            L.check(L.TIMER.launch("bev_dynamic_flow", lambda: lib.liso_bev_dynamic_mask_f32(
+                L.ptr(pts), pts.shape[-1], L.ptr(val), L.ptr(coors), L.ptr(fl), fl.shape[-1], L.ptr(ome), B, N, h, w, L.ptr(th),
+                int(th.dtype == torch.float64), float(dynamic_thresh_scale), L.ptr(dyn), L.ptr(nrf), L.ptr(mask), L.ptr(ws), nbytes,
+                L.stream_ptr())), "bev_dynamic_flow")
+        return dyn, nrf, mask
     with torch.cuda.device(dev):
         L.check(L.TIMER.launch("bev_dynamic_flow", lambda: lib.liso_bev_dynamic_flow_f32(
             L.ptr(pts), pts.shape[-1], L.ptr(val), L.ptr(coors), L.ptr(fl), fl.shape[-1], L.ptr(ome), B, N, h, w,
```

Result: no change. 1016 (-0.0%).
